# microsoft/vision-longformer

Hardware: NVIDIA H100
Metric: images/sec ViL-Small 224x224 training (higher is better)
Workload: dtype bf16

## Files before the change

### include/vil_attn.h

```cpp
#ifndef VIL_ATTN_H_
#define VIL_ATTN_H_

#include <stdint.h>

#ifdef __cplusplus
extern "C" {
#endif

#define VIL_ATTN_ABI_VERSION 3

enum { VIL_F32 = 0, VIL_BF16 = 1, VIL_F16 = 2 };

enum {
  VIL_IMPL_AUTO    = 0,
  VIL_IMPL_SIMT    = 1,
  VIL_IMPL_WGMMA   = 2
};

enum {
  VIL_FLAG_F32_OUT = 1,
  VIL_FLAG_UNFUSED = 2
};

enum {
  VIL_OK = 0,
  VIL_E_BADARG = -1,
  VIL_E_UNSUPPORTED = -2,
  VIL_E_CUDA = -3,
  VIL_E_WORKSPACE = -4
};

typedef struct VilTensor4 {
  void*   ptr;
  int64_t sb, sh, st;
} VilTensor4;

typedef struct VilAttnParams {
  int32_t struct_bytes;
  int32_t dtype;
  int32_t impl;
  int32_t B, H, D;
  int32_t nx, ny;
  int32_t w;
  int32_t nglo;
  int32_t exact;
  int32_t mode;
  float   scale;
  int32_t skip_mask;
  int32_t flags;

  VilTensor4 q;
  VilTensor4 k, v;
  VilTensor4 qg;
  VilTensor4 kg, vg;
  VilTensor4 o;
  VilTensor4 og;
  float* lse;
  float* lse_g;
  const float* bias_table;
  const float* g2l;
  const float* g2g;

  VilTensor4 d_o, d_og;
  VilTensor4 dq, dk, dv;
  VilTensor4 dqg;
  VilTensor4 dkg, dvg;
  float* d_bias_table;
  float* d_g2l;
  float* d_g2g;

  void*   workspace;
  int64_t workspace_bytes;

  float    dropout_p;
  uint32_t reserved2;
  uint64_t dropout_seed;
  uint64_t dropout_offset;
} VilAttnParams;

int         vil_attn_abi_version(void);
const char* vil_attn_last_error(void);
int64_t     vil_attn_launch_count(void);
const char* vil_attn_last_impl(void);
const char* vil_attn_last_kernel(void);

int64_t vil_attn_workspace_bytes(const VilAttnParams* p, int backward);

int vil_attn_wgmma_supported(const VilAttnParams* p);

int vil_attn_fwd_sm100(const VilAttnParams* p, void* stream);

int vil_attn_bwd_sm100(const VilAttnParams* p, void* stream);

typedef struct VilLayerNormParams {
  int32_t struct_bytes;
  int32_t x_dtype;
  int32_t y_dtype;
  int32_t C;
  int64_t rows;
  float   eps;
  int32_t reserved;
  const void*  x;
  const float* gamma;
  const float* beta;
  void*        y;
  float*       mean;
  float*       rstd;
  const void*  dy;
  void*        dx;
  float*       dgamma;
  float*       dbeta;
  void*        workspace;
  int64_t      workspace_bytes;
} VilLayerNormParams;

int64_t vil_layernorm_workspace_bytes(const VilLayerNormParams* p);
int vil_layernorm_fwd_sm100(const VilLayerNormParams* p, void* stream);
int vil_layernorm_bwd_sm100(const VilLayerNormParams* p, void* stream);

typedef struct VilAddNormParams {
  int32_t struct_bytes;
  int32_t b_dtype;
  int32_t y_dtype;
  int32_t C;
  int64_t rows;
  int64_t rows_per_sample;
  float   eps;
  int32_t reserved;
  const float* x;
  const void*  br;
  const float* bias;
  const float* rowscale;
  const float* gamma;
  const float* beta;
  float*       xo;
  void*        y;
  float*       mean;
  float*       rstd;
  const void*  dy;
  const float* gres;
  float*       dx;
  void*        dbr;
  float*       dgamma;
  float*       dbeta;
  float*       dbias;
  void*        workspace;
  int64_t      workspace_bytes;
} VilAddNormParams;

int64_t vil_addnorm_workspace_bytes(const VilAddNormParams* p);
int vil_addnorm_fwd_sm100(const VilAddNormParams* p, void* stream);
int vil_addnorm_bwd_sm100(const VilAddNormParams* p, void* stream);

enum { VIL_ACT_NONE = 0, VIL_ACT_GELU = 1 };
typedef struct VilBiasActParams {
  int32_t struct_bytes;
  int32_t dtype;
  int32_t C;
  int32_t act;
  int64_t rows;
  const void*  z;
  const float* bias;
  void*        a;
  const void*  da;
  void*        dz;
  float*       dbias;
  void*        workspace;
  int64_t      workspace_bytes;
} VilBiasActParams;

int64_t vil_bias_act_workspace_bytes(const VilBiasActParams* p);
int vil_bias_act_fwd_sm100(const VilBiasActParams* p, void* stream);
int vil_bias_act_bwd_sm100(const VilBiasActParams* p, void* stream);

#ifdef __cplusplus
}
#endif
#endif
```

### vision_longformer_b200/_lib.py

```python
from __future__ import annotations

import ctypes
import os
import threading

_HERE = os.path.dirname(os.path.abspath(__file__))
LIB_NAME = "libvil_attn.so"
LIB_PATH = os.environ.get("VIL_ATTN_LIB") or os.path.join(_HERE, LIB_NAME)

VIL_F32, VIL_BF16, VIL_F16 = 0, 1, 2
VIL_IMPL_AUTO, VIL_IMPL_SIMT, VIL_IMPL_WGMMA = 0, 1, 2
VIL_E_BADARG, VIL_E_UNSUPPORTED, VIL_E_CUDA, VIL_E_WORKSPACE = -1, -2, -3, -4
ABI_VERSION = 3
VIL_FLAG_F32_OUT, VIL_FLAG_UNFUSED = 1, 2

EXPORTS = (
    "vil_attn_abi_version", "vil_attn_last_error", "vil_attn_launch_count", "vil_attn_last_impl", "vil_attn_last_kernel",
    "vil_attn_workspace_bytes", "vil_attn_wgmma_supported", "vil_attn_fwd_sm100", "vil_attn_bwd_sm100",
    "vil_layernorm_workspace_bytes", "vil_layernorm_fwd_sm100", "vil_layernorm_bwd_sm100",
    "vil_addnorm_workspace_bytes", "vil_addnorm_fwd_sm100", "vil_addnorm_bwd_sm100",
    "vil_bias_act_workspace_bytes", "vil_bias_act_fwd_sm100", "vil_bias_act_bwd_sm100",
)
VIL_ACT_NONE, VIL_ACT_GELU = 0, 1


class VilTensor4(ctypes.Structure):
    _fields_ = [("ptr", ctypes.c_void_p), ("sb", ctypes.c_int64), ("sh", ctypes.c_int64), ("st", ctypes.c_int64)]


class VilAttnParams(ctypes.Structure):
    _fields_ = [
        ("struct_bytes", ctypes.c_int32), ("dtype", ctypes.c_int32), ("impl", ctypes.c_int32),
        ("B", ctypes.c_int32), ("H", ctypes.c_int32), ("D", ctypes.c_int32),
        ("nx", ctypes.c_int32), ("ny", ctypes.c_int32), ("w", ctypes.c_int32), ("nglo", ctypes.c_int32),
        ("exact", ctypes.c_int32), ("mode", ctypes.c_int32), ("scale", ctypes.c_float), ("skip_mask", ctypes.c_int32),
        ("flags", ctypes.c_int32),
        ("q", VilTensor4), ("k", VilTensor4), ("v", VilTensor4),
        ("qg", VilTensor4), ("kg", VilTensor4), ("vg", VilTensor4),
        ("o", VilTensor4), ("og", VilTensor4),
        ("lse", ctypes.c_void_p), ("lse_g", ctypes.c_void_p),
        ("bias_table", ctypes.c_void_p), ("g2l", ctypes.c_void_p), ("g2g", ctypes.c_void_p),
        ("d_o", VilTensor4), ("d_og", VilTensor4),
        ("dq", VilTensor4), ("dk", VilTensor4), ("dv", VilTensor4),
        ("dqg", VilTensor4), ("dkg", VilTensor4), ("dvg", VilTensor4),
        ("d_bias_table", ctypes.c_void_p), ("d_g2l", ctypes.c_void_p), ("d_g2g", ctypes.c_void_p),
        ("workspace", ctypes.c_void_p), ("workspace_bytes", ctypes.c_int64),
        ("dropout_p", ctypes.c_float), ("reserved2", ctypes.c_uint32),
        ("dropout_seed", ctypes.c_uint64), ("dropout_offset", ctypes.c_uint64),
    ]


class VilLayerNormParams(ctypes.Structure):
    _fields_ = [
        ("struct_bytes", ctypes.c_int32), ("x_dtype", ctypes.c_int32), ("y_dtype", ctypes.c_int32), ("C", ctypes.c_int32),
        ("rows", ctypes.c_int64), ("eps", ctypes.c_float), ("reserved", ctypes.c_int32),
        ("x", ctypes.c_void_p), ("gamma", ctypes.c_void_p), ("beta", ctypes.c_void_p),
        ("y", ctypes.c_void_p), ("mean", ctypes.c_void_p), ("rstd", ctypes.c_void_p),
        ("dy", ctypes.c_void_p), ("dx", ctypes.c_void_p), ("dgamma", ctypes.c_void_p), ("dbeta", ctypes.c_void_p),
        ("workspace", ctypes.c_void_p), ("workspace_bytes", ctypes.c_int64),
    ]


class VilAddNormParams(ctypes.Structure):
    _fields_ = [
        ("struct_bytes", ctypes.c_int32), ("b_dtype", ctypes.c_int32), ("y_dtype", ctypes.c_int32), ("C", ctypes.c_int32),
        ("rows", ctypes.c_int64), ("rows_per_sample", ctypes.c_int64), ("eps", ctypes.c_float), ("reserved", ctypes.c_int32),
        ("x", ctypes.c_void_p), ("br", ctypes.c_void_p), ("bias", ctypes.c_void_p), ("rowscale", ctypes.c_void_p),
        ("gamma", ctypes.c_void_p), ("beta", ctypes.c_void_p), ("xo", ctypes.c_void_p), ("y", ctypes.c_void_p),
        ("mean", ctypes.c_void_p), ("rstd", ctypes.c_void_p), ("dy", ctypes.c_void_p), ("gres", ctypes.c_void_p),
        ("dx", ctypes.c_void_p), ("dbr", ctypes.c_void_p), ("dgamma", ctypes.c_void_p), ("dbeta", ctypes.c_void_p),
        ("dbias", ctypes.c_void_p), ("workspace", ctypes.c_void_p), ("workspace_bytes", ctypes.c_int64),
    ]


class VilBiasActParams(ctypes.Structure):
    _fields_ = [
        ("struct_bytes", ctypes.c_int32), ("dtype", ctypes.c_int32), ("C", ctypes.c_int32), ("act", ctypes.c_int32),
        ("rows", ctypes.c_int64),
        ("z", ctypes.c_void_p), ("bias", ctypes.c_void_p), ("a", ctypes.c_void_p), ("da", ctypes.c_void_p),
        ("dz", ctypes.c_void_p), ("dbias", ctypes.c_void_p), ("workspace", ctypes.c_void_p), ("workspace_bytes", ctypes.c_int64),
    ]


_lib = None
_lock = threading.Lock()


def load() -> ctypes.CDLL:
    global _lib
    if _lib is not None:
        return _lib
    with _lock:
        if _lib is not None:
            return _lib
        if not os.path.exists(LIB_PATH):
            raise RuntimeError(
                f"{LIB_PATH} is missing: build it with `python -c 'import __graft_entry__ as g; g.build()'` "
                "(nvcc -gencode arch=compute_90a,code=sm_90a).  There is no CPU / PyTorch fallback.")
        lib = ctypes.CDLL(LIB_PATH)
        lib.vil_attn_abi_version.restype = ctypes.c_int
        lib.vil_attn_last_error.restype = ctypes.c_char_p
        lib.vil_attn_last_impl.restype = ctypes.c_char_p
        lib.vil_attn_last_kernel.restype = ctypes.c_char_p
        lib.vil_attn_launch_count.restype = ctypes.c_int64
        lib.vil_attn_workspace_bytes.restype = ctypes.c_int64
        lib.vil_attn_workspace_bytes.argtypes = [ctypes.POINTER(VilAttnParams), ctypes.c_int]
        lib.vil_attn_wgmma_supported.restype = ctypes.c_int
        lib.vil_attn_wgmma_supported.argtypes = [ctypes.POINTER(VilAttnParams)]
        for fn in (lib.vil_attn_fwd_sm100, lib.vil_attn_bwd_sm100):
            fn.restype = ctypes.c_int
            fn.argtypes = [ctypes.POINTER(VilAttnParams), ctypes.c_void_p]
        lib.vil_layernorm_workspace_bytes.restype = ctypes.c_int64
        lib.vil_layernorm_workspace_bytes.argtypes = [ctypes.POINTER(VilLayerNormParams)]
        for fn in (lib.vil_layernorm_fwd_sm100, lib.vil_layernorm_bwd_sm100):
            fn.restype = ctypes.c_int
            fn.argtypes = [ctypes.POINTER(VilLayerNormParams), ctypes.c_void_p]
        for ws, fns, st in ((lib.vil_addnorm_workspace_bytes, (lib.vil_addnorm_fwd_sm100, lib.vil_addnorm_bwd_sm100), VilAddNormParams),
                            (lib.vil_bias_act_workspace_bytes, (lib.vil_bias_act_fwd_sm100, lib.vil_bias_act_bwd_sm100), VilBiasActParams)):
            ws.restype = ctypes.c_int64
            ws.argtypes = [ctypes.POINTER(st)]
            for fn in fns:
                fn.restype = ctypes.c_int
                fn.argtypes = [ctypes.POINTER(st), ctypes.c_void_p]
        if lib.vil_attn_abi_version() != ABI_VERSION:
            raise RuntimeError(f"ABI mismatch: library {lib.vil_attn_abi_version()}, binding {ABI_VERSION}")
        _lib = lib
    return _lib


def last_error() -> str:
    return load().vil_attn_last_error().decode()


def last_impl() -> str:
    return load().vil_attn_last_impl().decode()


def last_kernel() -> str:
    return load().vil_attn_last_kernel().decode()


def launch_count() -> int:
    return int(load().vil_attn_launch_count())


def raise_for(code: int):
    if code == 0:
        return
    msg = last_error()
    if code == VIL_E_BADARG:
        raise ValueError(msg)
    if code == VIL_E_UNSUPPORTED:
        raise NotImplementedError(msg)
    raise RuntimeError(f"vil_attn error {code}: {msg}")
```

### vision_longformer_b200/csrc/vil_attn_api.cu

```cuda
#include <atomic>
#include <cmath>
#include <cstdarg>
#include <cstdio>
#include <cstring>

#include "vil_host.cuh"
#include "vil_layernorm.cuh"

namespace {

thread_local char g_err[512] = "";
thread_local const char* g_last_impl = "none";
thread_local const char* g_last_kernel = "";
std::atomic<long long> g_launches{0};

int fail(int code, const char* fmt, ...) {
  va_list ap;
  va_start(ap, fmt);
  vsnprintf(g_err, sizeof(g_err), fmt, ap);
  va_end(ap);
  return code;
}

#define VIL_CUDA_OK(expr)                                                                  \
  do {                                                                                     \
    cudaError_t e__ = (expr);                                                              \
    if (e__ != cudaSuccess) return fail(VIL_E_CUDA, "%s: %s", #expr, cudaGetErrorString(e__)); \
  } while (0)

#define VIL_LAUNCHED() g_launches.fetch_add(1, std::memory_order_relaxed)

int make_geo(const VilAttnParams* p, vil::Geo* g) {
  if (p == nullptr) return fail(VIL_E_BADARG, "params is NULL");
  if (p->struct_bytes != (int32_t)sizeof(VilAttnParams))
    return fail(VIL_E_BADARG, "VilAttnParams size mismatch: caller %d, library %d (ABI drift)", p->struct_bytes,
                (int)sizeof(VilAttnParams));
  if (p->dtype != VIL_F32 && p->dtype != VIL_BF16 && p->dtype != VIL_F16)
    return fail(VIL_E_BADARG, "dtype must be VIL_F32, VIL_BF16 or VIL_F16");
  if (p->B <= 0 || p->H <= 0 || p->D <= 0 || p->nx <= 0 || p->ny <= 0 || p->w <= 0 || p->nglo < 0)
    return fail(VIL_E_BADARG, "B, H, D, nx, ny, w must be positive and nglo non-negative");
  if (p->exact != 0 && p->exact != 1 && p->exact != -1)
    return fail(VIL_E_BADARG, "longsc exact should be in [0,1,-1]!");
  if (p->mode < -1 || p->mode > 8) return fail(VIL_E_BADARG, "mode must be in [-1, 8]");
  if (p->flags & ~(VIL_FLAG_F32_OUT | VIL_FLAG_UNFUSED)) return fail(VIL_E_BADARG, "unknown bits in flags");
  if ((p->flags & VIL_FLAG_F32_OUT) && p->dtype == VIL_F32)
    return fail(VIL_E_BADARG, "VIL_FLAG_F32_OUT is the parity build of the bf16 / fp16 kernels; dtype is already fp32");
  if (p->exact == 1 && p->mode != 0)
    return fail(VIL_E_BADARG, "exact sliding window (exact=1) only supports mode=0");
  if (p->D > 128) return fail(VIL_E_UNSUPPORTED, "head dim %d > 128 is not supported", p->D);
  if (p->w > 48) return fail(VIL_E_UNSUPPORTED, "window %d > 48 is not supported", p->w);
  if ((long long)p->nx * p->ny + p->nglo > 0x7fffffffLL / 4) return fail(VIL_E_UNSUPPORTED, "too many tokens");
  memset(g, 0, sizeof(*g));
  g->B = p->B; g->H = p->H; g->D = p->D;
  g->nx = p->nx; g->ny = p->ny; g->w = p->w; g->g = p->nglo; g->exact = p->exact; g->mode = p->mode;
  g->padx = (p->w - p->nx % p->w) % p->w;
  g->pady = (p->w - p->ny % p->w) % p->w;
  g->mx = (p->nx + g->padx) / p->w;
  g->my = (p->ny + g->pady) / p->w;
  g->Nloc = p->nx * p->ny;
  g->N = g->Nloc + p->nglo;
  g->w2 = p->w * p->w;
  g->npc = (g->w2 + 63) / 64;
  static const int o9[9][2] = {{-1, -1}, {-1, 0}, {-1, 1}, {0, -1}, {0, 0}, {0, 1}, {1, -1}, {1, 0}, {1, 1}};
  static const int om[9][2] = {{0, 0}, {-1, -1}, {-1, 0}, {-1, 1}, {0, -1}, {0, 1}, {1, -1}, {1, 0}, {1, 1}};
  if (p->mode == 0) {
    g->noffs = 9;
    for (int i = 0; i < 9; ++i) { g->offR[i] = o9[i][0]; g->offC[i] = o9[i][1]; }
  } else if (p->mode == -1) {
    g->noffs = 1;
  } else {
    g->noffs = 2;
    g->offR[1] = om[p->mode][0]; g->offC[1] = om[p->mode][1];
  }
  g->has_bias = p->bias_table != nullptr;
  g->scale = p->scale;
  if (g->has_bias && p->nglo > 0 && (p->g2l == nullptr || p->g2g == nullptr))
    return fail(VIL_E_BADARG, "bias_table given but g2l / g2g missing while nglo > 0");
  if (!g->has_bias && (p->g2l != nullptr || p->g2g != nullptr))
    return fail(VIL_E_BADARG, "g2l / g2g given without bias_table (rpe parameters come together)");
  if (!(p->dropout_p >= 0.f && p->dropout_p < 1.f))
    return fail(VIL_E_BADARG, "dropout_p must be in [0, 1) (got %g)", (double)p->dropout_p);
  g->drop_p = p->dropout_p;
  g->drop_scale = 1.0f / (1.0f - p->dropout_p);
  const double t = std::floor((double)p->dropout_p * 4294967296.0);
  g->drop_thresh = t >= 4294967295.0 ? 0xffffffffu : (uint32_t)t;
  g->seed_lo = (uint32_t)(p->dropout_seed & 0xffffffffu);
  g->seed_hi = (uint32_t)(p->dropout_seed >> 32);
  g->drop_off = (uint32_t)p->dropout_offset;
  return VIL_OK;
}

int check_tensor(const VilTensor4& t, const char* name) {
  if (t.ptr == nullptr) return fail(VIL_E_BADARG, "tensor %s is NULL", name);
  return VIL_OK;
}

int check_common(const VilAttnParams* p, const vil::Geo& g, bool bwd) {
  int rc;
  if ((rc = check_tensor(p->q, "q")) || (rc = check_tensor(p->k, "k")) || (rc = check_tensor(p->v, "v")) ||
      (rc = check_tensor(p->o, "o")))
    return rc;
  if (p->lse == nullptr) return fail(VIL_E_BADARG, "lse is NULL");
  if (g.g > 0) {
    if ((rc = check_tensor(p->qg, "qg")) || (rc = check_tensor(p->kg, "kg")) || (rc = check_tensor(p->vg, "vg")) ||
        (rc = check_tensor(p->og, "og")))
      return rc;
    if (p->lse_g == nullptr) return fail(VIL_E_BADARG, "lse_g is NULL");
  }
  if (bwd) {
    if ((rc = check_tensor(p->d_o, "d_o")) || (rc = check_tensor(p->dq, "dq")) || (rc = check_tensor(p->dk, "dk")) ||
        (rc = check_tensor(p->dv, "dv")))
      return rc;
    if (g.g > 0) {
      if ((rc = check_tensor(p->d_og, "d_og")) || (rc = check_tensor(p->dqg, "dqg"))) return rc;
      const bool shared = (p->kg.ptr == p->k.ptr) && (p->vg.ptr == p->v.ptr);
      if (!shared && ((rc = check_tensor(p->dkg, "dkg")) || (rc = check_tensor(p->dvg, "dvg")))) return rc;
    }
    const long long need = vil_attn_workspace_bytes(p, 1);
    if (p->workspace == nullptr || p->workspace_bytes < need)
      return fail(VIL_E_WORKSPACE, "workspace too small: need %lld bytes, got %lld", need,
                  (long long)p->workspace_bytes);
    if (g.has_bias && p->d_bias_table == nullptr) return fail(VIL_E_BADARG, "bias_table given but d_bias_table is NULL");
  }
  return VIL_OK;
}

int run(const VilAttnParams* p, void* stream, bool bwd) {
  vil::Geo g;
  int rc = make_geo(p, &g);
  if (rc) return rc;
  if ((rc = check_common(p, g, bwd))) return rc;
  cudaStream_t s = static_cast<cudaStream_t>(stream);
  const int tc_ok = vil::tc_supported(p, g, bwd);
  int impl = p->impl;
  if (impl == VIL_IMPL_AUTO) impl = tc_ok ? VIL_IMPL_WGMMA : VIL_IMPL_SIMT;
  if (impl == VIL_IMPL_WGMMA) {
    if (!tc_ok) return fail(VIL_E_UNSUPPORTED, "the wgmma family does not cover this configuration: %s", vil::tc_why_not(p, g, bwd));
    rc = bwd ? vil::tc_backward(p, g, s) : vil::tc_forward(p, g, s);
    if (rc == VIL_OK) g_last_impl = "wgmma";
    return rc;
  }
  if (impl != VIL_IMPL_SIMT) return fail(VIL_E_BADARG, "impl must be VIL_IMPL_AUTO, _SIMT or _TCGEN05");
  rc = vil::simt_run(p, g, s, bwd);
  if (rc == VIL_OK) g_last_impl = "simt";
  return rc;
}

}

namespace vil {
int shared_fail(int code, const char* msg) { return fail(code, "%s", msg); }
void count_launch() { VIL_LAUNCHED(); }
void note_kernel(const char* name) { g_last_kernel = name; }
}

namespace {

constexpr int kSMs = 132;

inline int ln_bwd_grid(long long rows) {
  long long g = rows / (vil::ln::kWarpsPerCta * 16);
  if (g < kSMs) g = kSMs;
  if (g > kSMs * 8) g = kSMs * 8;
  return (int)g;
}

int ln_check(const VilLayerNormParams* p, bool bwd) {
  if (p == nullptr) return fail(VIL_E_BADARG, "params is NULL");
  if (p->struct_bytes != (int32_t)sizeof(VilLayerNormParams)) return fail(VIL_E_BADARG, "VilLayerNormParams size mismatch");
  if (p->C <= 0 || p->C > 1024) return fail(VIL_E_UNSUPPORTED, "LayerNorm supports 1 <= C <= 1024 (got %d)", p->C);
  if (p->rows < 0) return fail(VIL_E_BADARG, "rows must be >= 0");
  const bool same = p->x_dtype == p->y_dtype;
  const bool mixed = p->x_dtype == VIL_F32 && (p->y_dtype == VIL_BF16 || p->y_dtype == VIL_F16);
  const bool widen = (p->x_dtype == VIL_BF16 || p->x_dtype == VIL_F16) && p->y_dtype == VIL_F32;
  if (!(same || mixed || widen) || p->x_dtype < 0 || p->x_dtype > 2) return fail(VIL_E_UNSUPPORTED, "unsupported LayerNorm dtype pair");
  if (!p->x || !p->gamma || !p->beta || !p->mean || !p->rstd) return fail(VIL_E_BADARG, "LayerNorm: NULL tensor");
  if (!bwd && !p->y) return fail(VIL_E_BADARG, "LayerNorm: y is NULL");
  if (bwd) {
    if (!p->dy || !p->dx || !p->dgamma || !p->dbeta) return fail(VIL_E_BADARG, "LayerNorm backward: NULL tensor");
    if (!p->workspace || p->workspace_bytes < vil_layernorm_workspace_bytes(p))
      return fail(VIL_E_WORKSPACE, "LayerNorm workspace too small");
  }
  return VIL_OK;
}

template <typename TX, typename TY, int NPL>
int ln_launch(const VilLayerNormParams* p, cudaStream_t s, bool bwd) {
  if (p->rows == 0) return VIL_OK;
  if (!bwd) {
    long long ctas = (p->rows + vil::ln::kWarpsPerCta - 1) / vil::ln::kWarpsPerCta;
    if (ctas > kSMs * 8) ctas = kSMs * 8;
    vil::ln::layernorm_fwd<TX, TY, NPL><<<(unsigned)ctas, vil::ln::kWarpsPerCta * 32, 0, s>>>(
        static_cast<const TX*>(p->x), p->gamma, p->beta, static_cast<TY*>(p->y), p->mean, p->rstd, p->rows, p->C, p->eps);
    VIL_LAUNCHED();
  } else {
    float* partial = static_cast<float*>(p->workspace);
    const int grid = ln_bwd_grid(p->rows);
    vil::ln::layernorm_bwd<TX, TY, NPL><<<grid, vil::ln::kWarpsPerCta * 32, 0, s>>>(
        static_cast<const TY*>(p->dy), static_cast<const TX*>(p->x), p->gamma, p->mean, p->rstd, static_cast<TX*>(p->dx),
        partial, p->rows, p->C);
    VIL_LAUNCHED();
    vil::ln::layernorm_bwd_reduce<<<(2 * p->C + 31) / 32, 256, 0, s>>>(partial, p->dgamma, p->dbeta, grid, p->C);
    VIL_LAUNCHED();
  }
  VIL_CUDA_OK(cudaGetLastError());
  return VIL_OK;
}

template <typename TX, typename TY>
int ln_dispatch_c(const VilLayerNormParams* p, cudaStream_t s, bool bwd) {
  const int npl = (p->C + 31) / 32;
  if (npl <= 3) return ln_launch<TX, TY, 3>(p, s, bwd);
  if (npl <= 6) return ln_launch<TX, TY, 6>(p, s, bwd);
  if (npl <= 12) return ln_launch<TX, TY, 12>(p, s, bwd);
  if (npl <= 24) return ln_launch<TX, TY, 24>(p, s, bwd);
  return ln_launch<TX, TY, 32>(p, s, bwd);
}

int ln_run(const VilLayerNormParams* p, void* stream, bool bwd) {
  int rc = ln_check(p, bwd);
  if (rc) return rc;
  cudaStream_t s = static_cast<cudaStream_t>(stream);
  if (p->x_dtype == VIL_F32) {
    if (p->y_dtype == VIL_F32) return ln_dispatch_c<float, float>(p, s, bwd);
    if (p->y_dtype == VIL_BF16) return ln_dispatch_c<float, __nv_bfloat16>(p, s, bwd);
    return ln_dispatch_c<float, __half>(p, s, bwd);
  }
  if (p->x_dtype == VIL_BF16)
    return p->y_dtype == VIL_F32 ? ln_dispatch_c<__nv_bfloat16, float>(p, s, bwd) : ln_dispatch_c<__nv_bfloat16, __nv_bfloat16>(p, s, bwd);
  return p->y_dtype == VIL_F32 ? ln_dispatch_c<__half, float>(p, s, bwd) : ln_dispatch_c<__half, __half>(p, s, bwd);
}

}

extern "C" {

int64_t vil_layernorm_workspace_bytes(const VilLayerNormParams* p) {
  if (p == nullptr || p->C <= 0) return VIL_E_BADARG;
  return (int64_t)ln_bwd_grid(p->rows) * 2 * p->C * 4 + 256;
}
int vil_layernorm_fwd_sm100(const VilLayerNormParams* p, void* stream) { return ln_run(p, stream, false); }
int vil_layernorm_bwd_sm100(const VilLayerNormParams* p, void* stream) { return ln_run(p, stream, true); }

#ifdef VIL_TRACE
int vil_attn_debug_set_trace(void* dev_ptr) {
  long long* p = static_cast<long long*>(dev_ptr);
  return (int)cudaMemcpyToSymbol(g_vil_trace, &p, sizeof(p));
}
#endif

int vil_attn_abi_version(void) { return VIL_ATTN_ABI_VERSION; }
const char* vil_attn_last_error(void) { return g_err; }
int64_t vil_attn_launch_count(void) { return g_launches.load(std::memory_order_relaxed); }
const char* vil_attn_last_impl(void) { return g_last_impl; }
const char* vil_attn_last_kernel(void) { return g_last_kernel; }

int64_t vil_attn_workspace_bytes(const VilAttnParams* p, int backward) {
  vil::Geo g;
  int rc = make_geo(p, &g);
  if (rc) return rc;
  long long bytes = 256;
  if (backward) bytes += vil::ws_floats(g) * 4;
  return bytes;
}

int vil_attn_wgmma_supported(const VilAttnParams* p) {
  vil::Geo g;
  int rc = make_geo(p, &g);
  if (rc) return rc;
  return vil::tc_supported(p, g, false) ? 1 : 0;
}

int vil_attn_fwd_sm100(const VilAttnParams* p, void* stream) { return run(p, stream, false); }
int vil_attn_bwd_sm100(const VilAttnParams* p, void* stream) { return run(p, stream, true); }

}
```

### vision_longformer_b200/csrc/vil_common.cuh

```cuda
#pragma once
#include <cuda_runtime.h>
#include <cuda_bf16.h>
#include <cuda_fp16.h>
#include <stdint.h>
#include "../../include/vil_attn.h"

namespace vil {

struct Geo {
  int B, H, D;
  int nx, ny, w, g, exact, mode;
  int padx, pady, mx, my;
  int Nloc, N, w2;
  int npc;
  int noffs;
  int offR[9], offC[9];
  int has_bias;
  float scale;
  float drop_p, drop_scale;
  uint32_t drop_thresh;
  uint32_t seed_lo, seed_hi, drop_off;
};

inline long long ws_off_delta_g(const Geo& g) { return ((long long)g.B * g.H * g.Nloc + 63) & ~63LL; }
inline long long ws_floats(const Geo& g) { return ws_off_delta_g(g) + (((long long)g.B * g.H * g.g + 63) & ~63LL); }

struct T4 {
  char* p;
  long long sb, sh, st;
};

template <typename T> struct ElemTraits;
template <> struct ElemTraits<float> {
  static __device__ __forceinline__ float to_f(float x) { return x; }
  static __device__ __forceinline__ float from_f(float x) { return x; }
};
template <> struct ElemTraits<__nv_bfloat16> {
  static __device__ __forceinline__ float to_f(__nv_bfloat16 x) { return __bfloat162float(x); }
  static __device__ __forceinline__ __nv_bfloat16 from_f(float x) { return __float2bfloat16_rn(x); }
};
template <> struct ElemTraits<__half> {
  static __device__ __forceinline__ float to_f(__half x) { return __half2float(x); }
  static __device__ __forceinline__ __half from_f(float x) { return __float2half_rn(x); }
};

template <typename T>
__device__ __forceinline__ const T* row_ptr(const T4& t, int b, int h, long long tok) {
  return reinterpret_cast<const T*>(t.p) + (long long)b * t.sb + (long long)h * t.sh + tok * t.st;
}
template <typename T>
__device__ __forceinline__ T* row_ptr_w(const T4& t, int b, int h, long long tok) {
  return reinterpret_cast<T*>(t.p) + (long long)b * t.sb + (long long)h * t.sh + tok * t.st;
}

template <typename T, int CNT>
__device__ __forceinline__ void load_seg(const T* __restrict__ row, int c0, int D, float (&r)[CNT]) {
  constexpr int PER16 = 16 / (int)sizeof(T);
  if constexpr (CNT % PER16 == 0) {
    if (c0 + CNT <= D && ((reinterpret_cast<uintptr_t>(row + c0)) & 15) == 0) {
#pragma unroll
      for (int v = 0; v < CNT / PER16; ++v) {
        int4 raw = __ldg(reinterpret_cast<const int4*>(row + c0) + v);
        const T* e = reinterpret_cast<const T*>(&raw);
#pragma unroll
        for (int u = 0; u < PER16; ++u) r[v * PER16 + u] = ElemTraits<T>::to_f(e[u]);
      }
      return;
    }
  }
#pragma unroll
  for (int c = 0; c < CNT; ++c) r[c] = (c0 + c < D) ? ElemTraits<T>::to_f(row[c0 + c]) : 0.f;
}

template <typename T, int CNT>
__device__ __forceinline__ void store_seg(T* __restrict__ row, int c0, int D, const float (&r)[CNT]) {
  constexpr int PER16 = 16 / (int)sizeof(T);
  if constexpr (CNT % PER16 == 0) {
    if (c0 + CNT <= D && ((reinterpret_cast<uintptr_t>(row + c0)) & 15) == 0) {
#pragma unroll
      for (int v = 0; v < CNT / PER16; ++v) {
        int4 raw;
        T* e = reinterpret_cast<T*>(&raw);
#pragma unroll
        for (int u = 0; u < PER16; ++u) e[u] = ElemTraits<T>::from_f(r[v * PER16 + u]);
        reinterpret_cast<int4*>(row + c0)[v] = raw;
      }
      return;
    }
  }
#pragma unroll
  for (int c = 0; c < CNT; ++c)
    if (c0 + c < D) row[c0 + c] = ElemTraits<T>::from_f(r[c]);
}

__device__ __forceinline__ uint4 philox(const Geo& g, uint32_t c0, uint32_t c1, uint32_t c2) {
  uint32_t x0 = c0, x1 = c1, x2 = c2, x3 = g.drop_off, k0 = g.seed_lo, k1 = g.seed_hi;
#pragma unroll
  for (int r = 0; r < 10; ++r) {
    const uint32_t lo0 = 0xD2511F53u * x0, hi0 = __umulhi(0xD2511F53u, x0);
    const uint32_t lo1 = 0xCD9E8D57u * x2, hi1 = __umulhi(0xCD9E8D57u, x2);
    x0 = hi1 ^ x1 ^ k0; x1 = lo1; x2 = hi0 ^ x3 ^ k1; x3 = lo0;
    k0 += 0x9E3779B9u; k1 += 0xBB67AE85u;
  }
  return make_uint4(x0, x1, x2, x3);
}
__device__ __forceinline__ uint32_t philox_word(const uint4& x, uint32_t w) {
  return w == 0 ? x.x : w == 1 ? x.y : w == 2 ? x.z : x.w;
}
__device__ __forceinline__ bool drop_keep(const Geo& g, uint32_t row, uint32_t col, uint32_t sid) {
  return philox_word(philox(g, col >> 2, row, sid), col & 3) >= g.drop_thresh;
}
__device__ __forceinline__ void drop_keep2(const Geo& g, uint32_t row, uint32_t col, uint32_t sid, bool& k0, bool& k1) {
  const uint4 x = philox(g, col >> 2, row, sid);
  const uint32_t w = col & 3;
  k0 = philox_word(x, w) >= g.drop_thresh;
  const uint32_t u1 = w == 3 ? philox(g, (col >> 2) + 1, row, sid).x : philox_word(x, w + 1);
  k1 = u1 >= g.drop_thresh;
}

__device__ __forceinline__ float warp_sum(float v) {
#pragma unroll
  for (int o = 16; o > 0; o >>= 1) v += __shfl_xor_sync(0xffffffffu, v, o);
  return v;
}

}
```

### vision_longformer_b200/csrc/vil_sm90.cuh

```cuda
#pragma once
#include <cuda_bf16.h>
#include <cuda_fp16.h>
#include <stdint.h>

namespace sm90 {

__device__ __forceinline__ uint32_t smem_u32(const void* p) { return (uint32_t)__cvta_generic_to_shared(p); }

__host__ __device__ constexpr int core_off(int r, int c, int K) { return (((r >> 3) * (K >> 3) + (c >> 3)) << 6) + ((r & 7) << 3) + (c & 7); }

__device__ __forceinline__ uint64_t make_desc(uint32_t addr, uint32_t lbo, uint32_t sbo) {
  return (uint64_t)((addr >> 4) & 0x3FFF) | (uint64_t)(lbo >> 4) << 16 | (uint64_t)(sbo >> 4) << 32;
}
__device__ __forceinline__ uint64_t desc(const void* tile, int K, int k16) {
  return make_desc(smem_u32(tile) + k16 * 256, 128, (K >> 3) * 128);
}
__device__ __forceinline__ uint64_t desc_mn(const void* tile, int N, int k16) {
  return make_desc(smem_u32(tile) + k16 * N * 32, N * 16, 128);
}

__device__ __forceinline__ void cp_async16(void* dst, const void* src, int n) {
  asm volatile("cp.async.cg.shared.global [%0], [%1], 16, %2;" ::"r"(smem_u32(dst)), "l"(src), "r"(n) : "memory");
}
__device__ __forceinline__ void cp_async4(void* dst, const void* src) {
  asm volatile("cp.async.ca.shared.global [%0], [%1], 4;" ::"r"(smem_u32(dst)), "l"(src) : "memory");
}
__device__ __forceinline__ void cp_async_commit() { asm volatile("cp.async.commit_group;" ::: "memory"); }
template <int N>
__device__ __forceinline__ void cp_async_wait() { asm volatile("cp.async.wait_group %0;" ::"n"(N) : "memory"); }

__device__ __forceinline__ void wg_fence() { asm volatile("wgmma.fence.sync.aligned;" ::: "memory"); }
__device__ __forceinline__ void wg_commit() { asm volatile("wgmma.commit_group.sync.aligned;" ::: "memory"); }
__device__ __forceinline__ void wg_wait0() { asm volatile("wgmma.wait_group.sync.aligned 0;" ::: "memory"); }
__device__ __forceinline__ void fence_proxy_async() { asm volatile("fence.proxy.async.shared::cta;" ::: "memory"); }
template <int R>
__device__ __forceinline__ void reg_fence(float (&d)[R]) {
#pragma unroll
  for (int i = 0; i < R; ++i) asm volatile("" : "+f"(d[i])::"memory");
}

__device__ __forceinline__ void wgmma_ss_bf16_n16(float (&d)[8], uint64_t a, uint64_t b, uint32_t acc) {
  asm volatile(
      "{\n\t.reg .pred p;\n\tsetp.ne.b32 p, %10, 0;\n\t"
      "wgmma.mma_async.sync.aligned.m64n16k16.f32.bf16.bf16 {%0,%1,%2,%3,%4,%5,%6,%7}, %8, %9, p, 1, 1, 0, 0;\n\t}"
      : "+f"(d[0]), "+f"(d[1]), "+f"(d[2]), "+f"(d[3]), "+f"(d[4]), "+f"(d[5]), "+f"(d[6]), "+f"(d[7])
      : "l"(a), "l"(b), "r"(acc));
}
__device__ __forceinline__ void wgmma_rs_bf16_n16(float (&d)[8], const uint32_t (&a)[4], uint64_t b, uint32_t acc) {
  asm volatile(
      "{\n\t.reg .pred p;\n\tsetp.ne.b32 p, %13, 0;\n\t"
      "wgmma.mma_async.sync.aligned.m64n16k16.f32.bf16.bf16 {%0,%1,%2,%3,%4,%5,%6,%7}, {%8,%9,%10,%11}, %12, p, 1, 1, 1;\n\t}"
      : "+f"(d[0]), "+f"(d[1]), "+f"(d[2]), "+f"(d[3]), "+f"(d[4]), "+f"(d[5]), "+f"(d[6]), "+f"(d[7])
      : "r"(a[0]), "r"(a[1]), "r"(a[2]), "r"(a[3]), "l"(b), "r"(acc));
}
__device__ __forceinline__ void wgmma_ss_f16_n16(float (&d)[8], uint64_t a, uint64_t b, uint32_t acc) {
  asm volatile(
      "{\n\t.reg .pred p;\n\tsetp.ne.b32 p, %10, 0;\n\t"
      "wgmma.mma_async.sync.aligned.m64n16k16.f32.f16.f16 {%0,%1,%2,%3,%4,%5,%6,%7}, %8, %9, p, 1, 1, 0, 0;\n\t}"
      : "+f"(d[0]), "+f"(d[1]), "+f"(d[2]), "+f"(d[3]), "+f"(d[4]), "+f"(d[5]), "+f"(d[6]), "+f"(d[7])
      : "l"(a), "l"(b), "r"(acc));
}
__device__ __forceinline__ void wgmma_rs_f16_n16(float (&d)[8], const uint32_t (&a)[4], uint64_t b, uint32_t acc) {
  asm volatile(
      "{\n\t.reg .pred p;\n\tsetp.ne.b32 p, %13, 0;\n\t"
      "wgmma.mma_async.sync.aligned.m64n16k16.f32.f16.f16 {%0,%1,%2,%3,%4,%5,%6,%7}, {%8,%9,%10,%11}, %12, p, 1, 1, 1;\n\t}"
      : "+f"(d[0]), "+f"(d[1]), "+f"(d[2]), "+f"(d[3]), "+f"(d[4]), "+f"(d[5]), "+f"(d[6]), "+f"(d[7])
      : "r"(a[0]), "r"(a[1]), "r"(a[2]), "r"(a[3]), "l"(b), "r"(acc));
}
__device__ __forceinline__ void wgmma_ss_bf16_n32(float (&d)[16], uint64_t a, uint64_t b, uint32_t acc) {
  asm volatile(
      "{\n\t.reg .pred p;\n\tsetp.ne.b32 p, %18, 0;\n\t"
      "wgmma.mma_async.sync.aligned.m64n32k16.f32.bf16.bf16 {%0,%1,%2,%3,%4,%5,%6,%7,%8,%9,%10,%11,%12,%13,%14,%15}, %16, %17, p, 1, 1, 0, 0;\n\t}"
      : "+f"(d[0]), "+f"(d[1]), "+f"(d[2]), "+f"(d[3]), "+f"(d[4]), "+f"(d[5]), "+f"(d[6]), "+f"(d[7]), "+f"(d[8]), "+f"(d[9]), "+f"(d[10]), "+f"(d[11]), "+f"(d[12]), "+f"(d[13]), "+f"(d[14]), "+f"(d[15])
      : "l"(a), "l"(b), "r"(acc));
}
__device__ __forceinline__ void wgmma_rs_bf16_n32(float (&d)[16], const uint32_t (&a)[4], uint64_t b, uint32_t acc) {
  asm volatile(
      "{\n\t.reg .pred p;\n\tsetp.ne.b32 p, %21, 0;\n\t"
      "wgmma.mma_async.sync.aligned.m64n32k16.f32.bf16.bf16 {%0,%1,%2,%3,%4,%5,%6,%7,%8,%9,%10,%11,%12,%13,%14,%15}, {%16,%17,%18,%19}, %20, p, 1, 1, 1;\n\t}"
      : "+f"(d[0]), "+f"(d[1]), "+f"(d[2]), "+f"(d[3]), "+f"(d[4]), "+f"(d[5]), "+f"(d[6]), "+f"(d[7]), "+f"(d[8]), "+f"(d[9]), "+f"(d[10]), "+f"(d[11]), "+f"(d[12]), "+f"(d[13]), "+f"(d[14]), "+f"(d[15])
      : "r"(a[0]), "r"(a[1]), "r"(a[2]), "r"(a[3]), "l"(b), "r"(acc));
}
__device__ __forceinline__ void wgmma_ss_f16_n32(float (&d)[16], uint64_t a, uint64_t b, uint32_t acc) {
  asm volatile(
      "{\n\t.reg .pred p;\n\tsetp.ne.b32 p, %18, 0;\n\t"
      "wgmma.mma_async.sync.aligned.m64n32k16.f32.f16.f16 {%0,%1,%2,%3,%4,%5,%6,%7,%8,%9,%10,%11,%12,%13,%14,%15}, %16, %17, p, 1, 1, 0, 0;\n\t}"
      : "+f"(d[0]), "+f"(d[1]), "+f"(d[2]), "+f"(d[3]), "+f"(d[4]), "+f"(d[5]), "+f"(d[6]), "+f"(d[7]), "+f"(d[8]), "+f"(d[9]), "+f"(d[10]), "+f"(d[11]), "+f"(d[12]), "+f"(d[13]), "+f"(d[14]), "+f"(d[15])
      : "l"(a), "l"(b), "r"(acc));
}
__device__ __forceinline__ void wgmma_rs_f16_n32(float (&d)[16], const uint32_t (&a)[4], uint64_t b, uint32_t acc) {
  asm volatile(
      "{\n\t.reg .pred p;\n\tsetp.ne.b32 p, %21, 0;\n\t"
      "wgmma.mma_async.sync.aligned.m64n32k16.f32.f16.f16 {%0,%1,%2,%3,%4,%5,%6,%7,%8,%9,%10,%11,%12,%13,%14,%15}, {%16,%17,%18,%19}, %20, p, 1, 1, 1;\n\t}"
      : "+f"(d[0]), "+f"(d[1]), "+f"(d[2]), "+f"(d[3]), "+f"(d[4]), "+f"(d[5]), "+f"(d[6]), "+f"(d[7]), "+f"(d[8]), "+f"(d[9]), "+f"(d[10]), "+f"(d[11]), "+f"(d[12]), "+f"(d[13]), "+f"(d[14]), "+f"(d[15])
      : "r"(a[0]), "r"(a[1]), "r"(a[2]), "r"(a[3]), "l"(b), "r"(acc));
}
__device__ __forceinline__ void wgmma_ss_bf16_n64(float (&d)[32], uint64_t a, uint64_t b, uint32_t acc) {
  asm volatile(
      "{\n\t.reg .pred p;\n\tsetp.ne.b32 p, %34, 0;\n\t"
      "wgmma.mma_async.sync.aligned.m64n64k16.f32.bf16.bf16 {%0,%1,%2,%3,%4,%5,%6,%7,%8,%9,%10,%11,%12,%13,%14,%15,%16,%17,%18,%19,%20,%21,%22,%23,%24,%25,%26,%27,%28,%29,%30,%31}, %32, %33, p, 1, 1, 0, 0;\n\t}"
      : "+f"(d[0]), "+f"(d[1]), "+f"(d[2]), "+f"(d[3]), "+f"(d[4]), "+f"(d[5]), "+f"(d[6]), "+f"(d[7]), "+f"(d[8]), "+f"(d[9]), "+f"(d[10]), "+f"(d[11]), "+f"(d[12]), "+f"(d[13]), "+f"(d[14]), "+f"(d[15]), "+f"(d[16]), "+f"(d[17]), "+f"(d[18]), "+f"(d[19]), "+f"(d[20]), "+f"(d[21]), "+f"(d[22]), "+f"(d[23]), "+f"(d[24]), "+f"(d[25]), "+f"(d[26]), "+f"(d[27]), "+f"(d[28]), "+f"(d[29]), "+f"(d[30]), "+f"(d[31])
      : "l"(a), "l"(b), "r"(acc));
}
__device__ __forceinline__ void wgmma_rs_bf16_n64(float (&d)[32], const uint32_t (&a)[4], uint64_t b, uint32_t acc) {
  asm volatile(
      "{\n\t.reg .pred p;\n\tsetp.ne.b32 p, %37, 0;\n\t"
      "wgmma.mma_async.sync.aligned.m64n64k16.f32.bf16.bf16 {%0,%1,%2,%3,%4,%5,%6,%7,%8,%9,%10,%11,%12,%13,%14,%15,%16,%17,%18,%19,%20,%21,%22,%23,%24,%25,%26,%27,%28,%29,%30,%31}, {%32,%33,%34,%35}, %36, p, 1, 1, 1;\n\t}"
      : "+f"(d[0]), "+f"(d[1]), "+f"(d[2]), "+f"(d[3]), "+f"(d[4]), "+f"(d[5]), "+f"(d[6]), "+f"(d[7]), "+f"(d[8]), "+f"(d[9]), "+f"(d[10]), "+f"(d[11]), "+f"(d[12]), "+f"(d[13]), "+f"(d[14]), "+f"(d[15]), "+f"(d[16]), "+f"(d[17]), "+f"(d[18]), "+f"(d[19]), "+f"(d[20]), "+f"(d[21]), "+f"(d[22]), "+f"(d[23]), "+f"(d[24]), "+f"(d[25]), "+f"(d[26]), "+f"(d[27]), "+f"(d[28]), "+f"(d[29]), "+f"(d[30]), "+f"(d[31])
      : "r"(a[0]), "r"(a[1]), "r"(a[2]), "r"(a[3]), "l"(b), "r"(acc));
}
__device__ __forceinline__ void wgmma_ss_f16_n64(float (&d)[32], uint64_t a, uint64_t b, uint32_t acc) {
  asm volatile(
      "{\n\t.reg .pred p;\n\tsetp.ne.b32 p, %34, 0;\n\t"
      "wgmma.mma_async.sync.aligned.m64n64k16.f32.f16.f16 {%0,%1,%2,%3,%4,%5,%6,%7,%8,%9,%10,%11,%12,%13,%14,%15,%16,%17,%18,%19,%20,%21,%22,%23,%24,%25,%26,%27,%28,%29,%30,%31}, %32, %33, p, 1, 1, 0, 0;\n\t}"
      : "+f"(d[0]), "+f"(d[1]), "+f"(d[2]), "+f"(d[3]), "+f"(d[4]), "+f"(d[5]), "+f"(d[6]), "+f"(d[7]), "+f"(d[8]), "+f"(d[9]), "+f"(d[10]), "+f"(d[11]), "+f"(d[12]), "+f"(d[13]), "+f"(d[14]), "+f"(d[15]), "+f"(d[16]), "+f"(d[17]), "+f"(d[18]), "+f"(d[19]), "+f"(d[20]), "+f"(d[21]), "+f"(d[22]), "+f"(d[23]), "+f"(d[24]), "+f"(d[25]), "+f"(d[26]), "+f"(d[27]), "+f"(d[28]), "+f"(d[29]), "+f"(d[30]), "+f"(d[31])
      : "l"(a), "l"(b), "r"(acc));
}
__device__ __forceinline__ void wgmma_rs_f16_n64(float (&d)[32], const uint32_t (&a)[4], uint64_t b, uint32_t acc) {
  asm volatile(
      "{\n\t.reg .pred p;\n\tsetp.ne.b32 p, %37, 0;\n\t"
      "wgmma.mma_async.sync.aligned.m64n64k16.f32.f16.f16 {%0,%1,%2,%3,%4,%5,%6,%7,%8,%9,%10,%11,%12,%13,%14,%15,%16,%17,%18,%19,%20,%21,%22,%23,%24,%25,%26,%27,%28,%29,%30,%31}, {%32,%33,%34,%35}, %36, p, 1, 1, 1;\n\t}"
      : "+f"(d[0]), "+f"(d[1]), "+f"(d[2]), "+f"(d[3]), "+f"(d[4]), "+f"(d[5]), "+f"(d[6]), "+f"(d[7]), "+f"(d[8]), "+f"(d[9]), "+f"(d[10]), "+f"(d[11]), "+f"(d[12]), "+f"(d[13]), "+f"(d[14]), "+f"(d[15]), "+f"(d[16]), "+f"(d[17]), "+f"(d[18]), "+f"(d[19]), "+f"(d[20]), "+f"(d[21]), "+f"(d[22]), "+f"(d[23]), "+f"(d[24]), "+f"(d[25]), "+f"(d[26]), "+f"(d[27]), "+f"(d[28]), "+f"(d[29]), "+f"(d[30]), "+f"(d[31])
      : "r"(a[0]), "r"(a[1]), "r"(a[2]), "r"(a[3]), "l"(b), "r"(acc));
}

template <typename T, int N> struct Wg;
#define VIL_WG(T, TN, N)                                                                                          \
  template <> struct Wg<T, N> {                                                                                   \
    static __device__ __forceinline__ void ss(float (&d)[N / 2], uint64_t a, uint64_t b, uint32_t acc) { wgmma_ss_##TN##_n##N(d, a, b, acc); } \
    static __device__ __forceinline__ void rs(float (&d)[N / 2], const uint32_t (&a)[4], uint64_t b, uint32_t acc) { wgmma_rs_##TN##_n##N(d, a, b, acc); } \
  };
VIL_WG(__nv_bfloat16, bf16, 16)
VIL_WG(__nv_bfloat16, bf16, 32)
VIL_WG(__nv_bfloat16, bf16, 64)
VIL_WG(__half, f16, 16)
VIL_WG(__half, f16, 32)
VIL_WG(__half, f16, 64)
#undef VIL_WG

template <typename T> __device__ __forceinline__ uint32_t pack2(float x, float y);
template <> __device__ __forceinline__ uint32_t pack2<__nv_bfloat16>(float x, float y) {
  __nv_bfloat162 v = __floats2bfloat162_rn(x, y);
  return *reinterpret_cast<uint32_t*>(&v);
}
template <> __device__ __forceinline__ uint32_t pack2<__half>(float x, float y) {
  __half2 v = __floats2half2_rn(x, y);
  return *reinterpret_cast<uint32_t*>(&v);
}

}
```

### vision_longformer_b200/csrc/vil_wgmma.cuh

```cuda
#pragma once
#include "vil_common.cuh"
#include "vil_sm90.cuh"

namespace vil {
namespace wg {

constexpr int kThreads = 128;

struct Cta { int b, h, R, C, piece; };

__device__ __forceinline__ Cta decode(const Geo& g, int bid) {
  Cta c;
  c.piece = bid % g.npc; bid /= g.npc;
  c.C = bid % g.my; bid /= g.my;
  c.R = bid % g.mx; bid /= g.mx;
  c.h = bid % g.H;
  c.b = bid / g.H;
  return c;
}

__device__ __forceinline__ int acc_row(int i) { return ((threadIdx.x >> 5) << 4) + ((threadIdx.x & 31) >> 2) + (((i >> 1) & 1) << 3); }
__device__ __forceinline__ int acc_col(int i) { return ((i >> 2) << 3) + ((threadIdx.x & 3) << 1) + (i & 1); }

constexpr int kStages = 3;

template <typename T, int HD>
__device__ __forceinline__ void stage_row(T* tile, const T* base, long long st, long long tok, int row, int half, int D) {
  constexpr int HH = HD / 2;
  const T* src = base + (tok < 0 ? 0 : tok * st);
#pragma unroll
  for (int g8 = 0; g8 < HH / 8; ++g8) {
    const int c = half * HH + g8 * 8;
    const bool in = tok >= 0 && c < D;
    sm90::cp_async16(tile + sm90::core_off(row, c, HD), in ? src + c : base, in ? 16 : 0);
  }
}

template <typename T>
__device__ __forceinline__ void to_a_frag(const float (&s)[32], int kk, uint32_t (&a)[4]) {
  a[0] = sm90::pack2<T>(s[8 * kk + 0], s[8 * kk + 1]);
  a[1] = sm90::pack2<T>(s[8 * kk + 2], s[8 * kk + 3]);
  a[2] = sm90::pack2<T>(s[8 * kk + 4], s[8 * kk + 5]);
  a[3] = sm90::pack2<T>(s[8 * kk + 6], s[8 * kk + 7]);
}

template <typename TO, int HD>
__device__ __forceinline__ void store_rows(const float (&acc)[HD / 2], int e, TO* row, int D, float mul) {
  const int c0 = (threadIdx.x & 3) << 1;
#pragma unroll
  for (int j = 0; j < HD / 8; ++j) {
    const int col = 8 * j + c0;
    if (col < D) row[col] = ElemTraits<TO>::from_f(acc[4 * j + 2 * e] * mul);
    if (col + 1 < D) row[col + 1] = ElemTraits<TO>::from_f(acc[4 * j + 2 * e + 1] * mul);
  }
}

__device__ __forceinline__ void drop_key_piece(float (&x)[32], const Geo& geo, const uint32_t (&row)[2], int cbase, uint32_t sid,
                                               float mul) {
  uint32_t keep = 0;
#pragma unroll 1
  for (int i = 0; i < 32; i += 2) {
    bool k0, k1;
    drop_keep2(geo, (i & 2) ? row[1] : row[0], (uint32_t)(cbase + acc_col(i)), sid, k0, k1);
    keep |= ((uint32_t)k0 | ((uint32_t)k1 << 1)) << i;
  }
#pragma unroll
  for (int i = 0; i < 32; ++i) x[i] = (keep >> i) & 1u ? x[i] * mul : 0.f;
}

__device__ __forceinline__ void drop_rows(const Geo& geo, int R, int C, int piece, uint32_t (&row)[2]) {
#pragma unroll
  for (int e = 0; e < 2; ++e) {
    const int l = piece * 64 + acc_row(2 * e);
    row[e] = (uint32_t)((R * geo.w + l / geo.w) * geo.ny + C * geo.w + l % geo.w);
  }
}

struct Visit {
  int r, c;
  int dR, dC;
  int cut;
  int oi;
};

__device__ __forceinline__ int visit_list(const Geo& geo, int R, int C, int sgn, Visit* vl) {
  int n = 0;
  for (int oi = 0; oi < geo.noffs; ++oi) {
    const int dR = geo.offR[oi], dC = geo.offC[oi];
    int r = R + sgn * dR, c = C + sgn * dC;
    if (geo.exact == -1) { r = (r + geo.mx) % geo.mx; c = (c + geo.my) % geo.my; }
    else if (r < 0 || r >= geo.mx || c < 0 || c >= geo.my) continue;
    const int qR = sgn > 0 ? R : r, qC = sgn > 0 ? C : c;
    if (threadIdx.x == 0) vl[n] = Visit{r, c, dR, dC, (qR + dR == geo.mx - 1) | ((qC + dC == geo.my - 1) << 1), oi};
    ++n;
  }
  return n;
}

__device__ __forceinline__ int drop_col_base(const Geo& geo, const Visit* vl, int ngp, int pi) {
  if (pi < ngp) return pi * 64;
  const int vi = (pi - ngp) / geo.npc;
  return geo.g + vl[vi].oi * geo.w2 + (pi - ngp - vi * geo.npc) * 64;
}

struct SlotWalk {
  int vi, pj, kr, kc;
  int r0, c0, dr, dc;
  __device__ __forceinline__ SlotWalk(const Geo& geo, int slot)
      : vi(0), pj(0), r0(slot / geo.w), c0(slot % geo.w), dr(64 / geo.w), dc(64 % geo.w) { kr = r0; kc = c0; }
  __device__ __forceinline__ void next(const Geo& geo) {
    if (++pj == geo.npc) { pj = 0; ++vi; kr = r0; kc = c0; return; }
    kr += dr; kc += dc;
    if (kc >= geo.w) { kc -= geo.w; ++kr; }
  }
};

__device__ __forceinline__ void chunk_key(const Geo& geo, const Visit& v, int kr, int kc, long long& tok, bool& ok, int& vr, int& vc) {
  const int w = geo.w;
  const int ar = v.r * w + kr, ac = v.c * w + kc;
  const bool real = (ar < geo.nx) && (ac < geo.ny);
  if (geo.exact == -1)
    ok = !(((v.cut & 1) && (kr >= w - geo.padx)) || ((v.cut & 2) && (kc >= w - geo.pady)));
  else
    ok = real;
  tok = (ok && real) ? geo.g + (long long)ar * geo.ny + ac : -1;
  vr = v.dR * w + kr; vc = v.dC * w + kc;
}

__device__ __forceinline__ void key_slot(const Geo& geo, const Visit* vl, int ngp, int pi, int slot, SlotWalk& wk, int& gk,
                                         long long& tok, bool& ok, int& vr, int& vc) {
  gk = -1; tok = -1; ok = false; vr = 0; vc = 0;
  if (pi < ngp) {
    const int t = pi * 64 + slot;
    if (t < geo.g) { gk = t; tok = t; ok = true; }
    return;
  }
  if (wk.kr < geo.w) chunk_key(geo, vl[wk.vi], wk.kr, wk.kc, tok, ok, vr, vc);
  wk.next(geo);
}

struct KeyCols {
  float* bias;
  int* tix;
  short* kr;
  short* kc;
};
struct QRows {
  int qr[2], qc[2];
  bool ok[2];
};

__device__ __forceinline__ QRows query_rows(const Geo& geo, int R, int C, int piece) {
  QRows q;
  const int w = geo.w;
#pragma unroll
  for (int e = 0; e < 2; ++e) {
    const int l = piece * 64 + acc_row(2 * e);
    const bool in = l < geo.w2;
    q.qr[e] = in ? l / w : 0; q.qc[e] = in ? l % w : 0;
    q.ok[e] = in && (R * w + q.qr[e] < geo.nx) && (C * w + q.qc[e] < geo.ny);
  }
  return q;
}

__device__ __forceinline__ void stage_key_cols(const Geo& geo, const KeyCols& kc, int h, const float* __restrict__ g2l, int gk,
                                               bool ok, int vr, int vc) {
  const int slot = threadIdx.x >> 1;
  float bias = ok ? 0.f : -INFINITY;
  if (gk >= 0 && geo.has_bias) bias = g2l[((long long)geo.H + h) * geo.g + gk];
  kc.bias[slot] = bias;
  kc.tix[slot] = vr * (4 * geo.w - 1) + vc;
  kc.kr[slot] = (short)vr;
  kc.kc[slot] = (short)vc;
}

__device__ __forceinline__ void row_tix(const Geo& geo, const QRows& q, int (&tb)[2]) {
  const int w = geo.w, tw = 4 * w - 1;
  tb[0] = (q.qr[0] + 2 * w - 1) * tw + q.qc[0] + 2 * w - 1;
  tb[1] = (q.qr[1] + 2 * w - 1) * tw + q.qc[1] + 2 * w - 1;
}

template <bool RPE, bool WIN>
__device__ __forceinline__ float key_score(const Geo& geo, const KeyCols& kc, const float* tab, const QRows& q, const int (&tb)[2],
                                           int e, int j, int gl, float s, int& bidx) {
  float bias = kc.bias[j];
  bidx = -1;
  if (RPE && j >= gl) { bidx = tb[e] - kc.tix[j]; bias += tab[bidx]; }
  if (WIN && (abs(q.qr[e] - kc.kr[j]) > geo.w || abs(q.qc[e] - kc.kc[j]) > geo.w)) return -INFINITY;
  return fmaf(geo.scale, s, bias);
}

__device__ __forceinline__ int key_epilogue(const Geo& geo) { return (geo.has_bias ? 2 : 0) | (geo.exact == 1 ? 1 : 0); }

template <bool RPE, bool WIN>
__device__ __forceinline__ void fwd_scores(float (&s)[32], float (&mx)[2], const Geo& geo, const KeyCols& kc, const float* tab,
                                           const QRows& q, int gl) {
  int tb[2] = {0, 0};
  if (RPE) row_tix(geo, q, tb);
#pragma unroll
  for (int i = 0; i < 32; ++i) {
    const int e = (i >> 1) & 1;
    int bidx;
    s[i] = key_score<RPE, WIN>(geo, kc, tab, q, tb, e, acc_col(i), gl, s[i], bidx);
    mx[e] = fmaxf(mx[e], s[i]);
  }
}

template <bool RPE, bool WIN>
__device__ __forceinline__ void dq_scores(float (&s)[32], const float (&dp)[32], const Geo& geo, const KeyCols& kc,
                                          const float* tab, const QRows& q, int gl, const float (&lse_r)[2],
                                          const float (&del_r)[2], float* __restrict__ d_table, int h) {
  int tb[2] = {0, 0};
  if (RPE) row_tix(geo, q, tb);
#pragma unroll
  for (int i = 0; i < 32; ++i) {
    const int e = (i >> 1) & 1;
    int bidx;
    const float val = key_score<RPE, WIN>(geo, kc, tab, q, tb, e, acc_col(i), gl, s[i], bidx);
    const float ds = __expf(val - lse_r[e]) * (dp[i] - del_r[e]);
    if (RPE && d_table != nullptr && bidx >= 0 && q.ok[e] && val != -INFINITY)
      atomicAdd(d_table + (long long)bidx * geo.H + h, ds);
    s[i] = ds;
  }
}

constexpr size_t kKeyCols = 64 * (4 + 4 + 2 + 2);
constexpr size_t kQueryCols = 64 * (4 + 4 + 4 + 2 + 2 + 1);
constexpr size_t kVisits = 9 * sizeof(Visit);
__host__ __device__ constexpr size_t query_cols_bytes(bool drop) { return kQueryCols + (drop ? 64 * sizeof(int) : 0); }

__device__ __forceinline__ KeyCols key_cols(unsigned char* meta, int stage) {
  KeyCols kc;
  kc.bias = reinterpret_cast<float*>(meta + stage * kKeyCols);
  kc.tix = reinterpret_cast<int*>(kc.bias + 64);
  kc.kr = reinterpret_cast<short*>(kc.tix + 64);
  kc.kc = kc.kr + 64;
  return kc;
}

template <int HD> struct FwdSmem {
  static constexpr size_t tiles = (1 + 2 * kStages) * 64 * HD * 2;
  static size_t total(int tabn) { return (tiles + kStages * kKeyCols + kVisits + (size_t)tabn * 4 + 15) & ~size_t(15); }
};
template <int HD> struct DqSmem {
  static constexpr size_t tiles = (2 + 2 * kStages) * 64 * HD * 2;
  static size_t total(int tabn) { return (tiles + kStages * kKeyCols + kVisits + (size_t)tabn * 4 + 15) & ~size_t(15); }
};
template <int HD> struct DkvSmem {
  static constexpr size_t tiles = (2 + 2 * kStages) * 64 * HD * 2;
  static size_t total(int tabn, bool drop = false) {
    return (tiles + kStages * query_cols_bytes(drop) + kVisits + 64 * sizeof(int) + (size_t)tabn * 4 + 15) & ~size_t(15);
  }
};

template <typename T, int HD>
__device__ __forceinline__ void issue_key_piece(const Geo& geo, int pi, int npieces, int ngp, const Visit* vl, SlotWalk& wk,
                                                T* ring, unsigned char* meta, const T* kb, long long kst, const T* vb,
                                                long long vst, int h, const float* __restrict__ g2l) {
  if (pi < npieces) {
    const int slot = threadIdx.x >> 1, half = threadIdx.x & 1, st = pi % kStages;
    int gk, vr, vc;
    long long tok;
    bool ok;
    key_slot(geo, vl, ngp, pi, slot, wk, gk, tok, ok, vr, vc);
    T* Ks = ring + st * 2 * 64 * HD;
    stage_row<T, HD>(Ks, kb, kst, tok, slot, half, geo.D);
    stage_row<T, HD>(Ks + 64 * HD, vb, vst, tok, slot, half, geo.D);
    if (half == 0) stage_key_cols(geo, key_cols(meta, st), h, g2l, gk, ok, vr, vc);
  }
  sm90::cp_async_commit();
}

__device__ __forceinline__ void ring_wait() {
  sm90::cp_async_wait<kStages - 2>();
  sm90::fence_proxy_async();
  __syncthreads();
}

template <typename T, int HD, typename TO, bool DROP = false>
__global__ void __launch_bounds__(kThreads, HD <= 32 ? 5 : 3)
wg_fwd_local(Geo geo, T4 q, T4 k, T4 v, T4 o, float* __restrict__ lse, const float* __restrict__ table,
             const float* __restrict__ g2l) {
  constexpr int HH = HD / 2, TILE = 64 * HD;
  using W64 = sm90::Wg<T, 64>;
  using WHD = sm90::Wg<T, HD>;
  extern __shared__ __align__(128) unsigned char smem_raw[];
  T* Qs = reinterpret_cast<T*>(smem_raw);
  T* ring = Qs + TILE;
  unsigned char* meta = reinterpret_cast<unsigned char*>(ring + 2 * kStages * TILE);
  Visit* vl = reinterpret_cast<Visit*>(meta + kStages * kKeyCols);
  float* tab = reinterpret_cast<float*>(vl + 9);
  const int tabn = geo.has_bias ? (4 * geo.w - 1) * (4 * geo.w - 1) : 0;

  const Cta cid = decode(geo, blockIdx.x);
  const int b = cid.b, h = cid.h, R = cid.R, C = cid.C;
  const int tid = threadIdx.x, slot = tid >> 1, half = tid & 1;
  const int w = geo.w, D = geo.D;
  for (int i = tid; i < tabn; i += kThreads) tab[i] = table[(long long)i * geo.H + h];
  {
    const int l = cid.piece * 64 + slot;
    const int r = R * w + l / w, c = C * w + l % w;
    const bool real = l < geo.w2 && r < geo.nx && c < geo.ny;
    stage_row<T, HD>(Qs, row_ptr<T>(q, b, h, 0), q.st, real ? (long long)r * geo.ny + c : -1, slot, half, D);
  }
  float m[2] = {-INFINITY, -INFINITY}, lsum[2] = {0.f, 0.f};
  float oacc[HH];
#pragma unroll
  for (int i = 0; i < HH; ++i) oacc[i] = 0.f;

  const int ngp = (geo.g + 63) / 64, npieces = ngp + visit_list(geo, R, C, 1, vl) * geo.npc;
  const int epi = key_epilogue(geo);
  const T* kb = row_ptr<T>(k, b, h, 0);
  const T* vb = row_ptr<T>(v, b, h, 0);
  SlotWalk wk(geo, slot);
  __syncthreads();
#pragma unroll
  for (int p = 0; p < kStages - 1; ++p)
    issue_key_piece<T, HD>(geo, p, npieces, ngp, vl, wk, ring, meta, kb, k.st, vb, v.st, h, g2l);
  for (int pi = 0; pi < npieces; ++pi) {
    ring_wait();
    issue_key_piece<T, HD>(geo, pi + kStages - 1, npieces, ngp, vl, wk, ring, meta, kb, k.st, vb, v.st, h, g2l);
    const int st = pi % kStages;
    const T* Ks = ring + st * 2 * TILE;
    const T* Vs = Ks + TILE;
    const KeyCols kcol = key_cols(meta, st);
    float s[32];
    sm90::wg_fence();
#pragma unroll
    for (int kk = 0; kk < HD / 16; ++kk) W64::ss(s, sm90::desc(Qs, HD, kk), sm90::desc(Ks, HD, kk), kk > 0);
    sm90::wg_commit();
    sm90::wg_wait0();
    sm90::reg_fence(s);
    float mx[2] = {-INFINITY, -INFINITY};
    const int gl = geo.g - pi * 64;
    switch (epi) {
      case 0: fwd_scores<false, false>(s, mx, geo, kcol, tab, query_rows(geo, R, C, cid.piece), gl); break;
      case 1: fwd_scores<false, true>(s, mx, geo, kcol, tab, query_rows(geo, R, C, cid.piece), gl); break;
      case 2: fwd_scores<true, false>(s, mx, geo, kcol, tab, query_rows(geo, R, C, cid.piece), gl); break;
      default: fwd_scores<true, true>(s, mx, geo, kcol, tab, query_rows(geo, R, C, cid.piece), gl); break;
    }
    float corr[2];
#pragma unroll
    for (int e = 0; e < 2; ++e) {
      mx[e] = fmaxf(mx[e], __shfl_xor_sync(0xffffffffu, mx[e], 1));
      mx[e] = fmaxf(mx[e], __shfl_xor_sync(0xffffffffu, mx[e], 2));
      const float mn = fmaxf(m[e], mx[e]);
      corr[e] = (mn == -INFINITY) ? 1.f : __expf(m[e] - mn);
      m[e] = mn;
      lsum[e] *= corr[e];
    }
#pragma unroll
    for (int i = 0; i < 32; ++i) {
      const int e = (i >> 1) & 1;
      const float p = (m[e] == -INFINITY) ? 0.f : __expf(s[i] - m[e]);
      s[i] = p;
      lsum[e] += p;
    }
#pragma unroll
    for (int i = 0; i < HH; ++i) oacc[i] *= corr[(i >> 1) & 1];
    if constexpr (DROP) {
      uint32_t drow[2];
      drop_rows(geo, R, C, cid.piece, drow);
      drop_key_piece(s, geo, drow, drop_col_base(geo, vl, ngp, pi), 2u * (uint32_t)(b * geo.H + h), 1.f);
    }
    uint32_t a[4][4];
#pragma unroll
    for (int kk = 0; kk < 4; ++kk) to_a_frag<T>(s, kk, a[kk]);
    sm90::wg_fence();
#pragma unroll
    for (int kk = 0; kk < 4; ++kk) WHD::rs(oacc, a[kk], sm90::desc_mn(Vs, HD, kk), 1);
    sm90::wg_commit();
    sm90::wg_wait0();
    sm90::reg_fence(oacc);
  }
  const QRows qrow = query_rows(geo, R, C, cid.piece);
#pragma unroll
  for (int e = 0; e < 2; ++e) {
    lsum[e] += __shfl_xor_sync(0xffffffffu, lsum[e], 1);
    lsum[e] += __shfl_xor_sync(0xffffffffu, lsum[e], 2);
    if (!qrow.ok[e]) continue;
    const long long tokq = (long long)(R * w + qrow.qr[e]) * geo.ny + (C * w + qrow.qc[e]);
    const float inv = lsum[e] > 0.f ? 1.f / lsum[e] : 0.f;
    store_rows<TO, HD>(oacc, e, row_ptr_w<TO>(o, b, h, tokq), D, DROP ? inv * geo.drop_scale : inv);
    if ((tid & 3) == 0) lse[((long long)b * geo.H + h) * geo.Nloc + tokq] = m[e] + logf(lsum[e]);
  }
}

template <typename T, int HD, typename TO, bool DROP = false>
__global__ void __launch_bounds__(kThreads)
wg_bwd_dq(Geo geo, T4 q, T4 k, T4 v, T4 d_o, T4 dq, const float* __restrict__ lse, const float* __restrict__ delta,
          const float* __restrict__ table, const float* __restrict__ g2l, float* __restrict__ d_table) {
  constexpr int HH = HD / 2, TILE = 64 * HD;
  using W64 = sm90::Wg<T, 64>;
  using WHD = sm90::Wg<T, HD>;
  extern __shared__ __align__(128) unsigned char smem_raw[];
  T* Qs = reinterpret_cast<T*>(smem_raw);
  T* Gs = Qs + TILE;
  T* ring = Gs + TILE;
  unsigned char* meta = reinterpret_cast<unsigned char*>(ring + 2 * kStages * TILE);
  Visit* vl = reinterpret_cast<Visit*>(meta + kStages * kKeyCols);
  float* tab = reinterpret_cast<float*>(vl + 9);
  const int tabn = geo.has_bias ? (4 * geo.w - 1) * (4 * geo.w - 1) : 0;

  const Cta cid = decode(geo, blockIdx.x);
  const int b = cid.b, h = cid.h, R = cid.R, C = cid.C;
  const int tid = threadIdx.x, slot = tid >> 1, half = tid & 1;
  const int w = geo.w, D = geo.D;
  const long long bh = (long long)b * geo.H + h;
  for (int i = tid; i < tabn; i += kThreads) tab[i] = table[(long long)i * geo.H + h];
  {
    const int l = cid.piece * 64 + slot;
    const int r = R * w + l / w, c = C * w + l % w;
    const long long tokq = (l < geo.w2 && r < geo.nx && c < geo.ny) ? (long long)r * geo.ny + c : -1;
    stage_row<T, HD>(Qs, row_ptr<T>(q, b, h, 0), q.st, tokq, slot, half, D);
    stage_row<T, HD>(Gs, row_ptr<T>(d_o, b, h, 0), d_o.st, tokq, slot, half, D);
  }
  const QRows qrow = query_rows(geo, R, C, cid.piece);
  float lse_r[2], del_r[2];
#pragma unroll
  for (int e = 0; e < 2; ++e) {
    lse_r[e] = INFINITY; del_r[e] = 0.f;
    if (qrow.ok[e]) {
      const long long tokq = (long long)(R * w + qrow.qr[e]) * geo.ny + (C * w + qrow.qc[e]);
      lse_r[e] = lse[bh * geo.Nloc + tokq];
      del_r[e] = delta[bh * geo.Nloc + tokq];
    }
  }
  float dqacc[HH];
#pragma unroll
  for (int i = 0; i < HH; ++i) dqacc[i] = 0.f;

  const int ngp = (geo.g + 63) / 64, npieces = ngp + visit_list(geo, R, C, 1, vl) * geo.npc;
  const int epi = key_epilogue(geo);
  const T* kb = row_ptr<T>(k, b, h, 0);
  const T* vb = row_ptr<T>(v, b, h, 0);
  SlotWalk wk(geo, slot);
  __syncthreads();
#pragma unroll
  for (int p = 0; p < kStages - 1; ++p)
    issue_key_piece<T, HD>(geo, p, npieces, ngp, vl, wk, ring, meta, kb, k.st, vb, v.st, h, g2l);
  for (int pi = 0; pi < npieces; ++pi) {
    ring_wait();
    issue_key_piece<T, HD>(geo, pi + kStages - 1, npieces, ngp, vl, wk, ring, meta, kb, k.st, vb, v.st, h, g2l);
    const int st = pi % kStages;
    const T* Ks = ring + st * 2 * TILE;
    const T* Vs = Ks + TILE;
    const KeyCols kcol = key_cols(meta, st);
    float s[32], dp[32];
    sm90::wg_fence();
#pragma unroll
    for (int kk = 0; kk < HD / 16; ++kk) W64::ss(s, sm90::desc(Qs, HD, kk), sm90::desc(Ks, HD, kk), kk > 0);
#pragma unroll
    for (int kk = 0; kk < HD / 16; ++kk) W64::ss(dp, sm90::desc(Gs, HD, kk), sm90::desc(Vs, HD, kk), kk > 0);
    sm90::wg_commit();
    sm90::wg_wait0();
    sm90::reg_fence(s);
    sm90::reg_fence(dp);
    const int gl = geo.g - pi * 64;
    if constexpr (DROP) {
      uint32_t drow[2];
      drop_rows(geo, R, C, cid.piece, drow);
      drop_key_piece(dp, geo, drow, drop_col_base(geo, vl, ngp, pi), 2u * (uint32_t)(b * geo.H + h), geo.drop_scale);
    }
    switch (epi) {
      case 0: dq_scores<false, false>(s, dp, geo, kcol, tab, qrow, gl, lse_r, del_r, d_table, h); break;
      case 1: dq_scores<false, true>(s, dp, geo, kcol, tab, qrow, gl, lse_r, del_r, d_table, h); break;
      case 2: dq_scores<true, false>(s, dp, geo, kcol, tab, qrow, gl, lse_r, del_r, d_table, h); break;
      default: dq_scores<true, true>(s, dp, geo, kcol, tab, qrow, gl, lse_r, del_r, d_table, h); break;
    }
    uint32_t a[4][4];
#pragma unroll
    for (int kk = 0; kk < 4; ++kk) to_a_frag<T>(s, kk, a[kk]);
    sm90::wg_fence();
#pragma unroll
    for (int kk = 0; kk < 4; ++kk) WHD::rs(dqacc, a[kk], sm90::desc_mn(Ks, HD, kk), 1);
    sm90::wg_commit();
    sm90::wg_wait0();
    sm90::reg_fence(dqacc);
  }
#pragma unroll
  for (int e = 0; e < 2; ++e) {
    if (!qrow.ok[e]) continue;
    const long long tokq = (long long)(R * w + qrow.qr[e]) * geo.ny + (C * w + qrow.qc[e]);
    store_rows<TO, HD>(dqacc, e, row_ptr_w<TO>(dq, b, h, tokq), D, geo.scale);
  }
}


struct QueryCols {
  float* lse;
  float* del;
  int* tix;
  short* qr;
  short* qc;
  unsigned char* cut;
  int* tok;
};
struct KRows {
  int kr[2], kc[2], tb[2];
  int cut[2];
  bool real[2];
};

__device__ __forceinline__ int key_pos(const Geo& geo, int piece, int row) {
  const int lk = piece * 64 + row;
  return lk < geo.w2 ? (lk / geo.w) | ((lk % geo.w) << 8) | (1 << 16) : 0;
}

__device__ __forceinline__ KRows key_rows(const Geo& geo, int KR, int KC, const int* kpos) {
  KRows k;
  const int w = geo.w, tw = 4 * w - 1;
#pragma unroll
  for (int e = 0; e < 2; ++e) {
    const int pos = kpos[acc_row(2 * e)];
    const bool in = pos >> 16;
    k.kr[e] = pos & 0xff; k.kc[e] = (pos >> 8) & 0xff;
    k.real[e] = in && (KR * w + k.kr[e] < geo.nx) && (KC * w + k.kc[e] < geo.ny);
    k.tb[e] = k.kr[e] * tw + k.kc[e] - (2 * w - 1) * (tw + 1);
    k.cut[e] = (k.kr[e] >= w - geo.padx) | ((k.kc[e] >= w - geo.pady) << 1);
  }
  return k;
}

__device__ __forceinline__ QueryCols query_cols(unsigned char* meta, int stage, int bytes) {
  QueryCols qc;
  qc.lse = reinterpret_cast<float*>(meta + stage * bytes);
  qc.del = qc.lse + 64;
  qc.tix = reinterpret_cast<int*>(qc.del + 64);
  qc.qr = reinterpret_cast<short*>(qc.tix + 64);
  qc.qc = qc.qr + 64;
  qc.cut = reinterpret_cast<unsigned char*>(qc.qc + 64);
  qc.tok = reinterpret_cast<int*>(qc.cut + 64);
  return qc;
}

template <typename T, int HD, bool DROP>
__device__ __forceinline__ void issue_query_piece(const Geo& geo, int qp, int npieces, const Visit* vl, SlotWalk& wk, T* ring,
                                                  unsigned char* meta, const T* qb, long long qst, const T* gb, long long gst,
                                                  const float* __restrict__ lse, const float* __restrict__ delta) {
  if (qp < npieces) {
    const int slot = threadIdx.x >> 1, half = threadIdx.x & 1, st = qp % kStages, w = geo.w;
    bool qv = false;
    long long tq = 0;
    int qa = 0, qb2 = 0, cut = 0;
    if (wk.kr < w) {
      const Visit vq = vl[wk.vi];
      const int r = vq.r * w + wk.kr, c = vq.c * w + wk.kc;
      qv = (r < geo.nx) && (c < geo.ny);
      tq = (long long)r * geo.ny + c;
      qa = wk.kr - vq.dR * w; qb2 = wk.kc - vq.dC * w; cut = vq.cut;
    }
    wk.next(geo);
    T* Qs = ring + st * 2 * 64 * HD;
    stage_row<T, HD>(Qs, qb, qst, qv ? tq : -1, slot, half, geo.D);
    stage_row<T, HD>(Qs + 64 * HD, gb, gst, qv ? tq : -1, slot, half, geo.D);
    if (half == 0) {
      const QueryCols qcol = query_cols(meta, st, (int)query_cols_bytes(DROP));
      if (qv) {
        sm90::cp_async4(qcol.lse + slot, lse + tq);
        sm90::cp_async4(qcol.del + slot, delta + tq);
      } else {
        qcol.lse[slot] = INFINITY;
        qcol.del[slot] = 0.f;
      }
      const int tw = 4 * w - 1;
      qcol.tix[slot] = qa * tw + qb2;
      qcol.qr[slot] = (short)qa; qcol.qc[slot] = (short)qb2;
      qcol.cut[slot] = (unsigned char)cut;
      if (DROP) qcol.tok[slot] = (int)tq;
    }
  }
  sm90::cp_async_commit();
}

__device__ __forceinline__ int query_epilogue(const Geo& geo) {
  return (geo.has_bias ? 3 : 0) + (geo.exact == 1 ? 1 : geo.exact == -1 ? 2 : 0);
}

template <bool RPE, int MASK>
__device__ __forceinline__ void dkv_probs(float (&s)[32], float (&dp)[32], const Geo& geo, const QueryCols& qc, const float* tab,
                                          const KRows& kr) {
#pragma unroll
  for (int i = 0; i < 32; ++i) {
    const int e = (i >> 1) & 1, j = acc_col(i);
    float x = fmaf(geo.scale, s[i], RPE ? tab[qc.tix[j] - kr.tb[e]] : 0.f) - qc.lse[j];
    if (MASK == 1 && (abs(qc.qr[j] - kr.kr[e]) > geo.w || abs(qc.qc[j] - kr.kc[e]) > geo.w)) x = -INFINITY;
    if (MASK == 2 && (qc.cut[j] & kr.cut[e])) x = -INFINITY;
    const float p = __expf(x);
    s[i] = p;
    dp[i] = p * (dp[i] - qc.del[j]);
  }
}

template <typename T, int HD, typename TO, bool DROP = false>
__global__ void __launch_bounds__(kThreads, (HD <= 32 ? 4 : 3) - (DROP ? 1 : 0))
wg_bwd_dkv(Geo geo, T4 q, T4 k, T4 v, T4 d_o, T4 dk, T4 dv, const float* __restrict__ lse, const float* __restrict__ delta,
           const float* __restrict__ table) {
  constexpr int HH = HD / 2, TILE = 64 * HD;
  using W64 = sm90::Wg<T, 64>;
  using WHD = sm90::Wg<T, HD>;
  extern __shared__ __align__(128) unsigned char smem_raw[];
  T* Ks = reinterpret_cast<T*>(smem_raw);
  T* Vs = Ks + TILE;
  T* ring = Vs + TILE;
  unsigned char* meta = reinterpret_cast<unsigned char*>(ring + 2 * kStages * TILE);
  const int cols = (int)query_cols_bytes(DROP);
  Visit* vl = reinterpret_cast<Visit*>(meta + kStages * cols);
  int* kpos = reinterpret_cast<int*>(vl + 9);
  float* tab = reinterpret_cast<float*>(kpos + 64);
  const int tw = 4 * geo.w - 1;
  const int tabn = geo.has_bias ? tw * tw : 0;

  const Cta cid = decode(geo, blockIdx.x);
  const int b = cid.b, h = cid.h, KR = cid.R, KC = cid.C;
  const int tid = threadIdx.x, slot = tid >> 1, half = tid & 1;
  const int w = geo.w, D = geo.D;
  const long long bh = (long long)b * geo.H + h;
  for (int i = tid; i < tabn; i += kThreads) tab[i] = table[(long long)i * geo.H + h];
  {
    const int lk = cid.piece * 64 + slot;
    const int ar = KR * w + lk / w, ac = KC * w + lk % w;
    const long long tokk = (lk < geo.w2 && ar < geo.nx && ac < geo.ny) ? geo.g + (long long)ar * geo.ny + ac : -1;
    stage_row<T, HD>(Ks, row_ptr<T>(k, b, h, 0), k.st, tokk, slot, half, D);
    stage_row<T, HD>(Vs, row_ptr<T>(v, b, h, 0), v.st, tokk, slot, half, D);
    if (half == 0) kpos[slot] = key_pos(geo, cid.piece, slot);
  }
  float dkacc[HH], dvacc[HH];
#pragma unroll
  for (int i = 0; i < HH; ++i) { dkacc[i] = 0.f; dvacc[i] = 0.f; }

  const int npieces = visit_list(geo, KR, KC, -1, vl) * geo.npc;
  const int epi = query_epilogue(geo);
  SlotWalk wk(geo, slot);
  __syncthreads();
#pragma unroll
  for (int p = 0; p < kStages - 1; ++p)
    issue_query_piece<T, HD, DROP>(geo, p, npieces, vl, wk, ring, meta, row_ptr<T>(q, b, h, 0), q.st,
                                   row_ptr<T>(d_o, b, h, 0), d_o.st, lse + bh * geo.Nloc, delta + bh * geo.Nloc);
  for (int qp = 0; qp < npieces; ++qp) {
    ring_wait();
    issue_query_piece<T, HD, DROP>(geo, qp + kStages - 1, npieces, vl, wk, ring, meta, row_ptr<T>(q, b, h, 0), q.st,
                                   row_ptr<T>(d_o, b, h, 0), d_o.st, lse + bh * geo.Nloc, delta + bh * geo.Nloc);
    const int st = qp % kStages;
    const T* Qs = ring + st * 2 * TILE;
    const T* Gs = Qs + TILE;
    const QueryCols qcol = query_cols(meta, st, cols);
    uint32_t keep = 0;
    if constexpr (DROP) {
      const int vi = qp / geo.npc;
      const uint32_t c0 = (uint32_t)(geo.g + vl[vi].oi * geo.w2 + cid.piece * 64), sid = 2u * (uint32_t)(b * geo.H + h);
#pragma unroll 1
      for (int i = 0; i < 32; ++i)
        keep |= (uint32_t)drop_keep(geo, (uint32_t)qcol.tok[acc_col(i)], c0 + (uint32_t)acc_row(i), sid) << i;
    }
    float s[32], dp[32];
    sm90::wg_fence();
#pragma unroll
    for (int kk = 0; kk < HD / 16; ++kk) W64::ss(s, sm90::desc(Ks, HD, kk), sm90::desc(Qs, HD, kk), kk > 0);
#pragma unroll
    for (int kk = 0; kk < HD / 16; ++kk) W64::ss(dp, sm90::desc(Vs, HD, kk), sm90::desc(Gs, HD, kk), kk > 0);
    sm90::wg_commit();
    sm90::wg_wait0();
    sm90::reg_fence(s);
    sm90::reg_fence(dp);
    if constexpr (DROP) {
#pragma unroll
      for (int i = 0; i < 32; ++i) dp[i] = (keep >> i) & 1u ? dp[i] * geo.drop_scale : 0.f;
    }
    switch (epi) {
      case 0: dkv_probs<false, 0>(s, dp, geo, qcol, tab, key_rows(geo, KR, KC, kpos)); break;
      case 1: dkv_probs<false, 1>(s, dp, geo, qcol, tab, key_rows(geo, KR, KC, kpos)); break;
      case 2: dkv_probs<false, 2>(s, dp, geo, qcol, tab, key_rows(geo, KR, KC, kpos)); break;
      case 3: dkv_probs<true, 0>(s, dp, geo, qcol, tab, key_rows(geo, KR, KC, kpos)); break;
      case 4: dkv_probs<true, 1>(s, dp, geo, qcol, tab, key_rows(geo, KR, KC, kpos)); break;
      default: dkv_probs<true, 2>(s, dp, geo, qcol, tab, key_rows(geo, KR, KC, kpos)); break;
    }
    if constexpr (DROP) {
#pragma unroll
      for (int i = 0; i < 32; ++i) s[i] = (keep >> i) & 1u ? s[i] * geo.drop_scale : 0.f;
    }
    uint32_t ap[4][4], ad[4][4];
#pragma unroll
    for (int kk = 0; kk < 4; ++kk) { to_a_frag<T>(s, kk, ap[kk]); to_a_frag<T>(dp, kk, ad[kk]); }
    sm90::wg_fence();
#pragma unroll
    for (int kk = 0; kk < 4; ++kk) WHD::rs(dvacc, ap[kk], sm90::desc_mn(Gs, HD, kk), 1);
#pragma unroll
    for (int kk = 0; kk < 4; ++kk) WHD::rs(dkacc, ad[kk], sm90::desc_mn(Qs, HD, kk), 1);
    sm90::wg_commit();
    sm90::wg_wait0();
    sm90::reg_fence(dvacc);
    sm90::reg_fence(dkacc);
  }
  const KRows krow = key_rows(geo, KR, KC, kpos);
#pragma unroll
  for (int e = 0; e < 2; ++e) {
    if (!krow.real[e]) continue;
    const long long tokk = geo.g + (long long)(KR * w + krow.kr[e]) * geo.ny + (KC * w + krow.kc[e]);
    store_rows<TO, HD>(dkacc, e, row_ptr_w<TO>(dk, b, h, tokk), D, geo.scale);
    store_rows<TO, HD>(dvacc, e, row_ptr_w<TO>(dv, b, h, tokk), D, 1.f);
  }
}

}
}
```

Before: 3805.

## Size wgmma N-width to actual piece width to skip padded columns

Adds wgmma ss variants for N=8 and N=56 and selects the MMA width per piece (global pieces, last partial pieces, windows of at most 56 tokens) instead of always using N=64. The padded rows and columns of the 64-wide tiles are no longer computed in the score and backward dK/dV GEMMs. It also trims the matching epilogue and dropout loops. A new FULL_PIECES flag restores the old fixed-64 behaviour. The change adds template instantiations and runtime switches, which raises code size and branch cost.

```diff
diff --git a/include/vil_attn.h b/include/vil_attn.h
--- a/include/vil_attn.h
+++ b/include/vil_attn.h
@@ -19,7 +19,8 @@
 
 enum {
   VIL_FLAG_F32_OUT = 1,
-  VIL_FLAG_UNFUSED = 2
+  VIL_FLAG_UNFUSED = 2,
+  VIL_FLAG_FULL_PIECES = 4
 };
 
 enum {
diff --git a/vision_longformer_b200/_lib.py b/vision_longformer_b200/_lib.py
--- a/vision_longformer_b200/_lib.py
+++ b/vision_longformer_b200/_lib.py
@@ -12,7 +12,7 @@
 VIL_IMPL_AUTO, VIL_IMPL_SIMT, VIL_IMPL_WGMMA = 0, 1, 2
 VIL_E_BADARG, VIL_E_UNSUPPORTED, VIL_E_CUDA, VIL_E_WORKSPACE = -1, -2, -3, -4
 ABI_VERSION = 3
-VIL_FLAG_F32_OUT, VIL_FLAG_UNFUSED = 1, 2
+VIL_FLAG_F32_OUT, VIL_FLAG_UNFUSED, VIL_FLAG_FULL_PIECES = 1, 2, 4
 
 EXPORTS = (
     "vil_attn_abi_version", "vil_attn_last_error", "vil_attn_launch_count", "vil_attn_last_impl", "vil_attn_last_kernel",
diff --git a/vision_longformer_b200/csrc/vil_attn_api.cu b/vision_longformer_b200/csrc/vil_attn_api.cu
--- a/vision_longformer_b200/csrc/vil_attn_api.cu
+++ b/vision_longformer_b200/csrc/vil_attn_api.cu
@@ -42,7 +42,7 @@
   if (p->exact != 0 && p->exact != 1 && p->exact != -1)
     return fail(VIL_E_BADARG, "longsc exact should be in [0,1,-1]!");
   if (p->mode < -1 || p->mode > 8) return fail(VIL_E_BADARG, "mode must be in [-1, 8]");
-  if (p->flags & ~(VIL_FLAG_F32_OUT | VIL_FLAG_UNFUSED)) return fail(VIL_E_BADARG, "unknown bits in flags");
+  if (p->flags & ~(VIL_FLAG_F32_OUT | VIL_FLAG_UNFUSED | VIL_FLAG_FULL_PIECES)) return fail(VIL_E_BADARG, "unknown bits in flags");
   if ((p->flags & VIL_FLAG_F32_OUT) && p->dtype == VIL_F32)
     return fail(VIL_E_BADARG, "VIL_FLAG_F32_OUT is the parity build of the bf16 / fp16 kernels; dtype is already fp32");
   if (p->exact == 1 && p->mode != 0)
@@ -73,6 +73,7 @@
     g->offR[1] = om[p->mode][0]; g->offC[1] = om[p->mode][1];
   }
   g->has_bias = p->bias_table != nullptr;
+  g->full_pieces = (p->flags & VIL_FLAG_FULL_PIECES) != 0;
   g->scale = p->scale;
   if (g->has_bias && p->nglo > 0 && (p->g2l == nullptr || p->g2g == nullptr))
     return fail(VIL_E_BADARG, "bias_table given but g2l / g2g missing while nglo > 0");
diff --git a/vision_longformer_b200/csrc/vil_common.cuh b/vision_longformer_b200/csrc/vil_common.cuh
--- a/vision_longformer_b200/csrc/vil_common.cuh
+++ b/vision_longformer_b200/csrc/vil_common.cuh
@@ -16,6 +16,7 @@
   int noffs;
   int offR[9], offC[9];
   int has_bias;
+  int full_pieces;
   float scale;
   float drop_p, drop_scale;
   uint32_t drop_thresh;
diff --git a/vision_longformer_b200/csrc/vil_sm90.cuh b/vision_longformer_b200/csrc/vil_sm90.cuh
--- a/vision_longformer_b200/csrc/vil_sm90.cuh
+++ b/vision_longformer_b200/csrc/vil_sm90.cuh
@@ -39,26 +39,52 @@
   for (int i = 0; i < R; ++i) asm volatile("" : "+f"(d[i])::"memory");
 }
 
-__device__ __forceinline__ void wgmma_ss_bf16_n16(float (&d)[8], uint64_t a, uint64_t b, uint32_t acc) {
-  asm volatile(
-      "{\n\t.reg .pred p;\n\tsetp.ne.b32 p, %10, 0;\n\t"
-      "wgmma.mma_async.sync.aligned.m64n16k16.f32.bf16.bf16 {%0,%1,%2,%3,%4,%5,%6,%7}, %8, %9, p, 1, 1, 0, 0;\n\t}"
-      : "+f"(d[0]), "+f"(d[1]), "+f"(d[2]), "+f"(d[3]), "+f"(d[4]), "+f"(d[5]), "+f"(d[6]), "+f"(d[7])
-      : "l"(a), "l"(b), "r"(acc));
-}
+#define VIL_ACC4(d, i) "+f"(d[i]), "+f"(d[i + 1]), "+f"(d[i + 2]), "+f"(d[i + 3])
+#define VIL_ACC_8(d) VIL_ACC4(d, 0)
+#define VIL_ACC_16(d) VIL_ACC_8(d), VIL_ACC4(d, 4)
+#define VIL_ACC_32(d) VIL_ACC_16(d), VIL_ACC4(d, 8), VIL_ACC4(d, 12)
+#define VIL_ACC_56(d) VIL_ACC_32(d), VIL_ACC4(d, 16), VIL_ACC4(d, 20), VIL_ACC4(d, 24)
+#define VIL_ACC_64(d) VIL_ACC_56(d), VIL_ACC4(d, 28)
+#define VIL_REG_8 "%3,%4,%5,%6"
+#define VIL_REG_16 VIL_REG_8 ",%7,%8,%9,%10"
+#define VIL_REG_32 VIL_REG_16 ",%11,%12,%13,%14,%15,%16,%17,%18"
+#define VIL_REG_56 VIL_REG_32 ",%19,%20,%21,%22,%23,%24,%25,%26,%27,%28,%29,%30"
+#define VIL_REG_64 VIL_REG_56 ",%31,%32,%33,%34"
+#define VIL_WGMMA_SS(TN, N)                                                                                         \
+  __device__ __forceinline__ void wgmma_ss_##TN##_n##N(float (&d)[N / 2], uint64_t a, uint64_t b, uint32_t acc) {  \
+    asm volatile("{\n\t.reg .pred p;\n\tsetp.ne.b32 p, %2, 0;\n\t"                                                 \
+                 "wgmma.mma_async.sync.aligned.m64n" #N "k16.f32." #TN "." #TN " {" VIL_REG_##N "}, %0, %1, p, 1, 1, 0, 0;\n\t}" \
+                 : "+l"(a), "+l"(b), "+r"(acc), VIL_ACC_##N(d));                                                    \
+  }
+VIL_WGMMA_SS(bf16, 8)
+VIL_WGMMA_SS(bf16, 16)
+VIL_WGMMA_SS(bf16, 32)
+VIL_WGMMA_SS(bf16, 56)
+VIL_WGMMA_SS(bf16, 64)
+VIL_WGMMA_SS(f16, 8)
+VIL_WGMMA_SS(f16, 16)
+VIL_WGMMA_SS(f16, 32)
+VIL_WGMMA_SS(f16, 56)
+VIL_WGMMA_SS(f16, 64)
+#undef VIL_WGMMA_SS
+#undef VIL_ACC4
+#undef VIL_ACC_8
+#undef VIL_ACC_16
+#undef VIL_ACC_32
+#undef VIL_ACC_56
+#undef VIL_ACC_64
+#undef VIL_REG_8
+#undef VIL_REG_16
+#undef VIL_REG_32
+#undef VIL_REG_56
+#undef VIL_REG_64
+
 __device__ __forceinline__ void wgmma_rs_bf16_n16(float (&d)[8], const uint32_t (&a)[4], uint64_t b, uint32_t acc) {
   asm volatile(
       "{\n\t.reg .pred p;\n\tsetp.ne.b32 p, %13, 0;\n\t"
       "wgmma.mma_async.sync.aligned.m64n16k16.f32.bf16.bf16 {%0,%1,%2,%3,%4,%5,%6,%7}, {%8,%9,%10,%11}, %12, p, 1, 1, 1;\n\t}"
       : "+f"(d[0]), "+f"(d[1]), "+f"(d[2]), "+f"(d[3]), "+f"(d[4]), "+f"(d[5]), "+f"(d[6]), "+f"(d[7])
       : "r"(a[0]), "r"(a[1]), "r"(a[2]), "r"(a[3]), "l"(b), "r"(acc));
-}
-__device__ __forceinline__ void wgmma_ss_f16_n16(float (&d)[8], uint64_t a, uint64_t b, uint32_t acc) {
-  asm volatile(
-      "{\n\t.reg .pred p;\n\tsetp.ne.b32 p, %10, 0;\n\t"
-      "wgmma.mma_async.sync.aligned.m64n16k16.f32.f16.f16 {%0,%1,%2,%3,%4,%5,%6,%7}, %8, %9, p, 1, 1, 0, 0;\n\t}"
-      : "+f"(d[0]), "+f"(d[1]), "+f"(d[2]), "+f"(d[3]), "+f"(d[4]), "+f"(d[5]), "+f"(d[6]), "+f"(d[7])
-      : "l"(a), "l"(b), "r"(acc));
 }
 __device__ __forceinline__ void wgmma_rs_f16_n16(float (&d)[8], const uint32_t (&a)[4], uint64_t b, uint32_t acc) {
   asm volatile(
@@ -67,26 +93,12 @@
       : "+f"(d[0]), "+f"(d[1]), "+f"(d[2]), "+f"(d[3]), "+f"(d[4]), "+f"(d[5]), "+f"(d[6]), "+f"(d[7])
       : "r"(a[0]), "r"(a[1]), "r"(a[2]), "r"(a[3]), "l"(b), "r"(acc));
 }
-__device__ __forceinline__ void wgmma_ss_bf16_n32(float (&d)[16], uint64_t a, uint64_t b, uint32_t acc) {
-  asm volatile(
-      "{\n\t.reg .pred p;\n\tsetp.ne.b32 p, %18, 0;\n\t"
-      "wgmma.mma_async.sync.aligned.m64n32k16.f32.bf16.bf16 {%0,%1,%2,%3,%4,%5,%6,%7,%8,%9,%10,%11,%12,%13,%14,%15}, %16, %17, p, 1, 1, 0, 0;\n\t}"
-      : "+f"(d[0]), "+f"(d[1]), "+f"(d[2]), "+f"(d[3]), "+f"(d[4]), "+f"(d[5]), "+f"(d[6]), "+f"(d[7]), "+f"(d[8]), "+f"(d[9]), "+f"(d[10]), "+f"(d[11]), "+f"(d[12]), "+f"(d[13]), "+f"(d[14]), "+f"(d[15])
-      : "l"(a), "l"(b), "r"(acc));
-}
 __device__ __forceinline__ void wgmma_rs_bf16_n32(float (&d)[16], const uint32_t (&a)[4], uint64_t b, uint32_t acc) {
   asm volatile(
       "{\n\t.reg .pred p;\n\tsetp.ne.b32 p, %21, 0;\n\t"
       "wgmma.mma_async.sync.aligned.m64n32k16.f32.bf16.bf16 {%0,%1,%2,%3,%4,%5,%6,%7,%8,%9,%10,%11,%12,%13,%14,%15}, {%16,%17,%18,%19}, %20, p, 1, 1, 1;\n\t}"
       : "+f"(d[0]), "+f"(d[1]), "+f"(d[2]), "+f"(d[3]), "+f"(d[4]), "+f"(d[5]), "+f"(d[6]), "+f"(d[7]), "+f"(d[8]), "+f"(d[9]), "+f"(d[10]), "+f"(d[11]), "+f"(d[12]), "+f"(d[13]), "+f"(d[14]), "+f"(d[15])
       : "r"(a[0]), "r"(a[1]), "r"(a[2]), "r"(a[3]), "l"(b), "r"(acc));
-}
-__device__ __forceinline__ void wgmma_ss_f16_n32(float (&d)[16], uint64_t a, uint64_t b, uint32_t acc) {
-  asm volatile(
-      "{\n\t.reg .pred p;\n\tsetp.ne.b32 p, %18, 0;\n\t"
-      "wgmma.mma_async.sync.aligned.m64n32k16.f32.f16.f16 {%0,%1,%2,%3,%4,%5,%6,%7,%8,%9,%10,%11,%12,%13,%14,%15}, %16, %17, p, 1, 1, 0, 0;\n\t}"
-      : "+f"(d[0]), "+f"(d[1]), "+f"(d[2]), "+f"(d[3]), "+f"(d[4]), "+f"(d[5]), "+f"(d[6]), "+f"(d[7]), "+f"(d[8]), "+f"(d[9]), "+f"(d[10]), "+f"(d[11]), "+f"(d[12]), "+f"(d[13]), "+f"(d[14]), "+f"(d[15])
-      : "l"(a), "l"(b), "r"(acc));
 }
 __device__ __forceinline__ void wgmma_rs_f16_n32(float (&d)[16], const uint32_t (&a)[4], uint64_t b, uint32_t acc) {
   asm volatile(
@@ -95,26 +107,12 @@
       : "+f"(d[0]), "+f"(d[1]), "+f"(d[2]), "+f"(d[3]), "+f"(d[4]), "+f"(d[5]), "+f"(d[6]), "+f"(d[7]), "+f"(d[8]), "+f"(d[9]), "+f"(d[10]), "+f"(d[11]), "+f"(d[12]), "+f"(d[13]), "+f"(d[14]), "+f"(d[15])
       : "r"(a[0]), "r"(a[1]), "r"(a[2]), "r"(a[3]), "l"(b), "r"(acc));
 }
-__device__ __forceinline__ void wgmma_ss_bf16_n64(float (&d)[32], uint64_t a, uint64_t b, uint32_t acc) {
-  asm volatile(
-      "{\n\t.reg .pred p;\n\tsetp.ne.b32 p, %34, 0;\n\t"
-      "wgmma.mma_async.sync.aligned.m64n64k16.f32.bf16.bf16 {%0,%1,%2,%3,%4,%5,%6,%7,%8,%9,%10,%11,%12,%13,%14,%15,%16,%17,%18,%19,%20,%21,%22,%23,%24,%25,%26,%27,%28,%29,%30,%31}, %32, %33, p, 1, 1, 0, 0;\n\t}"
-      : "+f"(d[0]), "+f"(d[1]), "+f"(d[2]), "+f"(d[3]), "+f"(d[4]), "+f"(d[5]), "+f"(d[6]), "+f"(d[7]), "+f"(d[8]), "+f"(d[9]), "+f"(d[10]), "+f"(d[11]), "+f"(d[12]), "+f"(d[13]), "+f"(d[14]), "+f"(d[15]), "+f"(d[16]), "+f"(d[17]), "+f"(d[18]), "+f"(d[19]), "+f"(d[20]), "+f"(d[21]), "+f"(d[22]), "+f"(d[23]), "+f"(d[24]), "+f"(d[25]), "+f"(d[26]), "+f"(d[27]), "+f"(d[28]), "+f"(d[29]), "+f"(d[30]), "+f"(d[31])
-      : "l"(a), "l"(b), "r"(acc));
-}
 __device__ __forceinline__ void wgmma_rs_bf16_n64(float (&d)[32], const uint32_t (&a)[4], uint64_t b, uint32_t acc) {
   asm volatile(
       "{\n\t.reg .pred p;\n\tsetp.ne.b32 p, %37, 0;\n\t"
       "wgmma.mma_async.sync.aligned.m64n64k16.f32.bf16.bf16 {%0,%1,%2,%3,%4,%5,%6,%7,%8,%9,%10,%11,%12,%13,%14,%15,%16,%17,%18,%19,%20,%21,%22,%23,%24,%25,%26,%27,%28,%29,%30,%31}, {%32,%33,%34,%35}, %36, p, 1, 1, 1;\n\t}"
       : "+f"(d[0]), "+f"(d[1]), "+f"(d[2]), "+f"(d[3]), "+f"(d[4]), "+f"(d[5]), "+f"(d[6]), "+f"(d[7]), "+f"(d[8]), "+f"(d[9]), "+f"(d[10]), "+f"(d[11]), "+f"(d[12]), "+f"(d[13]), "+f"(d[14]), "+f"(d[15]), "+f"(d[16]), "+f"(d[17]), "+f"(d[18]), "+f"(d[19]), "+f"(d[20]), "+f"(d[21]), "+f"(d[22]), "+f"(d[23]), "+f"(d[24]), "+f"(d[25]), "+f"(d[26]), "+f"(d[27]), "+f"(d[28]), "+f"(d[29]), "+f"(d[30]), "+f"(d[31])
       : "r"(a[0]), "r"(a[1]), "r"(a[2]), "r"(a[3]), "l"(b), "r"(acc));
-}
-__device__ __forceinline__ void wgmma_ss_f16_n64(float (&d)[32], uint64_t a, uint64_t b, uint32_t acc) {
-  asm volatile(
-      "{\n\t.reg .pred p;\n\tsetp.ne.b32 p, %34, 0;\n\t"
-      "wgmma.mma_async.sync.aligned.m64n64k16.f32.f16.f16 {%0,%1,%2,%3,%4,%5,%6,%7,%8,%9,%10,%11,%12,%13,%14,%15,%16,%17,%18,%19,%20,%21,%22,%23,%24,%25,%26,%27,%28,%29,%30,%31}, %32, %33, p, 1, 1, 0, 0;\n\t}"
-      : "+f"(d[0]), "+f"(d[1]), "+f"(d[2]), "+f"(d[3]), "+f"(d[4]), "+f"(d[5]), "+f"(d[6]), "+f"(d[7]), "+f"(d[8]), "+f"(d[9]), "+f"(d[10]), "+f"(d[11]), "+f"(d[12]), "+f"(d[13]), "+f"(d[14]), "+f"(d[15]), "+f"(d[16]), "+f"(d[17]), "+f"(d[18]), "+f"(d[19]), "+f"(d[20]), "+f"(d[21]), "+f"(d[22]), "+f"(d[23]), "+f"(d[24]), "+f"(d[25]), "+f"(d[26]), "+f"(d[27]), "+f"(d[28]), "+f"(d[29]), "+f"(d[30]), "+f"(d[31])
-      : "l"(a), "l"(b), "r"(acc));
 }
 __device__ __forceinline__ void wgmma_rs_f16_n64(float (&d)[32], const uint32_t (&a)[4], uint64_t b, uint32_t acc) {
   asm volatile(
@@ -125,18 +123,22 @@
 }
 
 template <typename T, int N> struct Wg;
-#define VIL_WG(T, TN, N)                                                                                          \
-  template <> struct Wg<T, N> {                                                                                   \
-    static __device__ __forceinline__ void ss(float (&d)[N / 2], uint64_t a, uint64_t b, uint32_t acc) { wgmma_ss_##TN##_n##N(d, a, b, acc); } \
-    static __device__ __forceinline__ void rs(float (&d)[N / 2], const uint32_t (&a)[4], uint64_t b, uint32_t acc) { wgmma_rs_##TN##_n##N(d, a, b, acc); } \
-  };
-VIL_WG(__nv_bfloat16, bf16, 16)
-VIL_WG(__nv_bfloat16, bf16, 32)
-VIL_WG(__nv_bfloat16, bf16, 64)
-VIL_WG(__half, f16, 16)
-VIL_WG(__half, f16, 32)
-VIL_WG(__half, f16, 64)
-#undef VIL_WG
+#define VIL_SS(TN, N) \
+  static __device__ __forceinline__ void ss(float (&d)[N / 2], uint64_t a, uint64_t b, uint32_t acc) { wgmma_ss_##TN##_n##N(d, a, b, acc); }
+#define VIL_RS(TN, N) \
+  static __device__ __forceinline__ void rs(float (&d)[N / 2], const uint32_t (&a)[4], uint64_t b, uint32_t acc) { wgmma_rs_##TN##_n##N(d, a, b, acc); }
+template <> struct Wg<__nv_bfloat16, 8> { VIL_SS(bf16, 8) };
+template <> struct Wg<__nv_bfloat16, 16> { VIL_SS(bf16, 16) VIL_RS(bf16, 16) };
+template <> struct Wg<__nv_bfloat16, 32> { VIL_SS(bf16, 32) VIL_RS(bf16, 32) };
+template <> struct Wg<__nv_bfloat16, 56> { VIL_SS(bf16, 56) };
+template <> struct Wg<__nv_bfloat16, 64> { VIL_SS(bf16, 64) VIL_RS(bf16, 64) };
+template <> struct Wg<__half, 8> { VIL_SS(f16, 8) };
+template <> struct Wg<__half, 16> { VIL_SS(f16, 16) VIL_RS(f16, 16) };
+template <> struct Wg<__half, 32> { VIL_SS(f16, 32) VIL_RS(f16, 32) };
+template <> struct Wg<__half, 56> { VIL_SS(f16, 56) };
+template <> struct Wg<__half, 64> { VIL_SS(f16, 64) VIL_RS(f16, 64) };
+#undef VIL_SS
+#undef VIL_RS
 
 template <typename T> __device__ __forceinline__ uint32_t pack2(float x, float y);
 template <> __device__ __forceinline__ uint32_t pack2<__nv_bfloat16>(float x, float y) {
diff --git a/vision_longformer_b200/csrc/vil_wgmma.cuh b/vision_longformer_b200/csrc/vil_wgmma.cuh
--- a/vision_longformer_b200/csrc/vil_wgmma.cuh
+++ b/vision_longformer_b200/csrc/vil_wgmma.cuh
@@ -36,13 +36,27 @@
   }
 }
 
-template <typename T>
-__device__ __forceinline__ void to_a_frag(const float (&s)[32], int kk, uint32_t (&a)[4]) {
+template <typename T, int NW>
+__device__ __forceinline__ void to_a_frag(const float (&s)[NW / 2], int kk, uint32_t (&a)[4]) {
   a[0] = sm90::pack2<T>(s[8 * kk + 0], s[8 * kk + 1]);
   a[1] = sm90::pack2<T>(s[8 * kk + 2], s[8 * kk + 3]);
-  a[2] = sm90::pack2<T>(s[8 * kk + 4], s[8 * kk + 5]);
-  a[3] = sm90::pack2<T>(s[8 * kk + 6], s[8 * kk + 7]);
-}
+  if (8 * kk + 4 < NW / 2) {
+    a[2] = sm90::pack2<T>(s[8 * kk + 4], s[8 * kk + 5]);
+    a[3] = sm90::pack2<T>(s[8 * kk + 6], s[8 * kk + 7]);
+  } else {
+    a[2] = 0u;
+    a[3] = 0u;
+  }
+}
+
+__device__ __forceinline__ int piece_width(int n) { return n <= 8 ? 8 : n <= 56 ? 56 : 64; }
+
+#define VIL_BY_WIDTH(nw, ROUND)                                                                                      \
+  switch (nw) {                                                                                                      \
+    case 8: ROUND(8); break;                                                                                         \
+    case 56: ROUND(56); break;                                                                                       \
+    default: ROUND(64); break;                                                                                       \
+  }
 
 template <typename TO, int HD>
 __device__ __forceinline__ void store_rows(const float (&acc)[HD / 2], int e, TO* row, int D, float mul) {
@@ -55,17 +69,18 @@
   }
 }
 
-__device__ __forceinline__ void drop_key_piece(float (&x)[32], const Geo& geo, const uint32_t (&row)[2], int cbase, uint32_t sid,
-                                               float mul) {
+template <int NW>
+__device__ __forceinline__ void drop_key_piece(float (&x)[NW / 2], const Geo& geo, const uint32_t (&row)[2], int cbase,
+                                               uint32_t sid, float mul) {
   uint32_t keep = 0;
 #pragma unroll 1
-  for (int i = 0; i < 32; i += 2) {
+  for (int i = 0; i < NW / 2; i += 2) {
     bool k0, k1;
     drop_keep2(geo, (i & 2) ? row[1] : row[0], (uint32_t)(cbase + acc_col(i)), sid, k0, k1);
     keep |= ((uint32_t)k0 | ((uint32_t)k1 << 1)) << i;
   }
 #pragma unroll
-  for (int i = 0; i < 32; ++i) x[i] = (keep >> i) & 1u ? x[i] * mul : 0.f;
+  for (int i = 0; i < NW / 2; ++i) x[i] = (keep >> i) & 1u ? x[i] * mul : 0.f;
 }
 
 __device__ __forceinline__ void drop_rows(const Geo& geo, int R, int C, int piece, uint32_t (&row)[2]) {
@@ -115,6 +130,11 @@
   }
 };
 
+__device__ __forceinline__ int issue_width(const Geo& geo, int pi, int ngp, const SlotWalk& wk) {
+  const int n = pi < ngp ? min(64, geo.g - 64 * pi) : wk.pj == geo.npc - 1 ? geo.w2 - 64 * (geo.npc - 1) : 64;
+  return geo.full_pieces ? 64 : piece_width(n);
+}
+
 __device__ __forceinline__ void chunk_key(const Geo& geo, const Visit& v, int kr, int kc, long long& tok, bool& ok, int& vr, int& vc) {
   const int w = geo.w;
   const int ar = v.r * w + kr, ac = v.c * w + kc;
@@ -192,13 +212,13 @@
 
 __device__ __forceinline__ int key_epilogue(const Geo& geo) { return (geo.has_bias ? 2 : 0) | (geo.exact == 1 ? 1 : 0); }
 
-template <bool RPE, bool WIN>
-__device__ __forceinline__ void fwd_scores(float (&s)[32], float (&mx)[2], const Geo& geo, const KeyCols& kc, const float* tab,
-                                           const QRows& q, int gl) {
+template <bool RPE, bool WIN, int NW>
+__device__ __forceinline__ void fwd_scores(float (&s)[NW / 2], float (&mx)[2], const Geo& geo, const KeyCols& kc,
+                                           const float* tab, const QRows& q, int gl) {
   int tb[2] = {0, 0};
   if (RPE) row_tix(geo, q, tb);
 #pragma unroll
-  for (int i = 0; i < 32; ++i) {
+  for (int i = 0; i < NW / 2; ++i) {
     const int e = (i >> 1) & 1;
     int bidx;
     s[i] = key_score<RPE, WIN>(geo, kc, tab, q, tb, e, acc_col(i), gl, s[i], bidx);
@@ -206,14 +226,14 @@
   }
 }
 
-template <bool RPE, bool WIN>
-__device__ __forceinline__ void dq_scores(float (&s)[32], const float (&dp)[32], const Geo& geo, const KeyCols& kc,
+template <bool RPE, bool WIN, int NW>
+__device__ __forceinline__ void dq_scores(float (&s)[NW / 2], const float (&dp)[NW / 2], const Geo& geo, const KeyCols& kc,
                                           const float* tab, const QRows& q, int gl, const float (&lse_r)[2],
                                           const float (&del_r)[2], float* __restrict__ d_table, int h) {
   int tb[2] = {0, 0};
   if (RPE) row_tix(geo, q, tb);
 #pragma unroll
-  for (int i = 0; i < 32; ++i) {
+  for (int i = 0; i < NW / 2; ++i) {
     const int e = (i >> 1) & 1;
     int bidx;
     const float val = key_score<RPE, WIN>(geo, kc, tab, q, tb, e, acc_col(i), gl, s[i], bidx);
@@ -227,6 +247,7 @@
 constexpr size_t kKeyCols = 64 * (4 + 4 + 2 + 2);
 constexpr size_t kQueryCols = 64 * (4 + 4 + 4 + 2 + 2 + 1);
 constexpr size_t kVisits = 9 * sizeof(Visit);
+constexpr size_t kWidths = kStages * sizeof(int);
 __host__ __device__ constexpr size_t query_cols_bytes(bool drop) { return kQueryCols + (drop ? 64 * sizeof(int) : 0); }
 
 __device__ __forceinline__ KeyCols key_cols(unsigned char* meta, int stage) {
@@ -240,11 +261,11 @@
 
 template <int HD> struct FwdSmem {
   static constexpr size_t tiles = (1 + 2 * kStages) * 64 * HD * 2;
-  static size_t total(int tabn) { return (tiles + kStages * kKeyCols + kVisits + (size_t)tabn * 4 + 15) & ~size_t(15); }
+  static size_t total(int tabn) { return (tiles + kStages * kKeyCols + kVisits + kWidths + (size_t)tabn * 4 + 15) & ~size_t(15); }
 };
 template <int HD> struct DqSmem {
   static constexpr size_t tiles = (2 + 2 * kStages) * 64 * HD * 2;
-  static size_t total(int tabn) { return (tiles + kStages * kKeyCols + kVisits + (size_t)tabn * 4 + 15) & ~size_t(15); }
+  static size_t total(int tabn) { return (tiles + kStages * kKeyCols + kVisits + kWidths + (size_t)tabn * 4 + 15) & ~size_t(15); }
 };
 template <int HD> struct DkvSmem {
   static constexpr size_t tiles = (2 + 2 * kStages) * 64 * HD * 2;
@@ -253,20 +274,22 @@
   }
 };
 
-template <typename T, int HD>
+template <typename T, int HD, bool KRS, bool TRIM = true>
 __device__ __forceinline__ void issue_key_piece(const Geo& geo, int pi, int npieces, int ngp, const Visit* vl, SlotWalk& wk,
-                                                T* ring, unsigned char* meta, const T* kb, long long kst, const T* vb,
-                                                long long vst, int h, const float* __restrict__ g2l) {
+                                                int* widths, T* ring, unsigned char* meta, const T* kb, long long kst,
+                                                const T* vb, long long vst, int h, const float* __restrict__ g2l) {
   if (pi < npieces) {
     const int slot = threadIdx.x >> 1, half = threadIdx.x & 1, st = pi % kStages;
+    const int nw = TRIM ? issue_width(geo, pi, ngp, wk) : 64, nrs = (nw + 15) & ~15;
+    if (threadIdx.x == 0) widths[st] = nw;
     int gk, vr, vc;
     long long tok;
     bool ok;
     key_slot(geo, vl, ngp, pi, slot, wk, gk, tok, ok, vr, vc);
     T* Ks = ring + st * 2 * 64 * HD;
-    stage_row<T, HD>(Ks, kb, kst, tok, slot, half, geo.D);
-    stage_row<T, HD>(Ks + 64 * HD, vb, vst, tok, slot, half, geo.D);
-    if (half == 0) stage_key_cols(geo, key_cols(meta, st), h, g2l, gk, ok, vr, vc);
+    if (slot < (KRS ? nrs : nw)) stage_row<T, HD>(Ks, kb, kst, tok, slot, half, geo.D);
+    if (slot < (KRS ? nw : nrs)) stage_row<T, HD>(Ks + 64 * HD, vb, vst, tok, slot, half, geo.D);
+    if (half == 0 && slot < nw) stage_key_cols(geo, key_cols(meta, st), h, g2l, gk, ok, vr, vc);
   }
   sm90::cp_async_commit();
 }
@@ -275,6 +298,64 @@
   sm90::cp_async_wait<kStages - 2>();
   sm90::fence_proxy_async();
   __syncthreads();
+}
+
+template <typename T, int HD, bool DROP, int NW>
+__device__ __forceinline__ void fwd_round(const Geo& geo, const T* Qs, const T* Ks, const T* Vs, const KeyCols& kcol,
+                                          const float* tab, int b, int h, int R, int C, int piece, int pi, int epi, int ngp,
+                                          const Visit* vl, float (&m)[2], float (&lsum)[2], float (&oacc)[HD / 2]) {
+  constexpr int HH = HD / 2;
+  using WHD = sm90::Wg<T, HD>;
+  float s[NW / 2];
+  sm90::wg_fence();
+#pragma unroll
+  for (int kk = 0; kk < HD / 16; ++kk)
+    sm90::Wg<T, NW>::ss(s, sm90::desc(Qs, HD, kk), sm90::desc(Ks, HD, kk), kk > 0);
+  sm90::wg_commit();
+  sm90::wg_wait0();
+  sm90::reg_fence(s);
+  float mx[2] = {-INFINITY, -INFINITY};
+  const int gl = geo.g - pi * 64;
+  switch (epi) {
+    case 0: fwd_scores<false, false, NW>(s, mx, geo, kcol, tab, query_rows(geo, R, C, piece), gl); break;
+    case 1: fwd_scores<false, true, NW>(s, mx, geo, kcol, tab, query_rows(geo, R, C, piece), gl); break;
+    case 2: fwd_scores<true, false, NW>(s, mx, geo, kcol, tab, query_rows(geo, R, C, piece), gl); break;
+    default: fwd_scores<true, true, NW>(s, mx, geo, kcol, tab, query_rows(geo, R, C, piece), gl); break;
+  }
+  float corr[2];
+#pragma unroll
+  for (int e = 0; e < 2; ++e) {
+    mx[e] = fmaxf(mx[e], __shfl_xor_sync(0xffffffffu, mx[e], 1));
+    mx[e] = fmaxf(mx[e], __shfl_xor_sync(0xffffffffu, mx[e], 2));
+    const float mn = fmaxf(m[e], mx[e]);
+    corr[e] = (mn == -INFINITY) ? 1.f : __expf(m[e] - mn);
+    m[e] = mn;
+    lsum[e] *= corr[e];
+  }
+#pragma unroll
+  for (int i = 0; i < NW / 2; ++i) {
+    const int e = (i >> 1) & 1;
+    const float p = (m[e] == -INFINITY) ? 0.f : __expf(s[i] - m[e]);
+    s[i] = p;
+    lsum[e] += p;
+  }
+#pragma unroll
+  for (int i = 0; i < HH; ++i) oacc[i] *= corr[(i >> 1) & 1];
+  if constexpr (DROP) {
+    uint32_t drow[2];
+    drop_rows(geo, R, C, piece, drow);
+    drop_key_piece<NW>(s, geo, drow, drop_col_base(geo, vl, ngp, pi), 2u * (uint32_t)(b * geo.H + h), 1.f);
+  }
+  constexpr int NK = (NW + 15) / 16;
+  uint32_t a[NK][4];
+#pragma unroll
+  for (int kk = 0; kk < NK; ++kk) to_a_frag<T, NW>(s, kk, a[kk]);
+  sm90::wg_fence();
+#pragma unroll
+  for (int kk = 0; kk < NK; ++kk) WHD::rs(oacc, a[kk], sm90::desc_mn(Vs, HD, kk), 1);
+  sm90::wg_commit();
+  sm90::wg_wait0();
+  sm90::reg_fence(oacc);
 }
 
 template <typename T, int HD, typename TO, bool DROP = false>
@@ -282,14 +363,14 @@
 wg_fwd_local(Geo geo, T4 q, T4 k, T4 v, T4 o, float* __restrict__ lse, const float* __restrict__ table,
              const float* __restrict__ g2l) {
   constexpr int HH = HD / 2, TILE = 64 * HD;
-  using W64 = sm90::Wg<T, 64>;
   using WHD = sm90::Wg<T, HD>;
   extern __shared__ __align__(128) unsigned char smem_raw[];
   T* Qs = reinterpret_cast<T*>(smem_raw);
   T* ring = Qs + TILE;
   unsigned char* meta = reinterpret_cast<unsigned char*>(ring + 2 * kStages * TILE);
   Visit* vl = reinterpret_cast<Visit*>(meta + kStages * kKeyCols);
-  float* tab = reinterpret_cast<float*>(vl + 9);
+  int* widths = reinterpret_cast<int*>(vl + 9);
+  float* tab = reinterpret_cast<float*>(widths + kStages);
   const int tabn = geo.has_bias ? (4 * geo.w - 1) * (4 * geo.w - 1) : 0;
 
   const Cta cid = decode(geo, blockIdx.x);
@@ -316,62 +397,18 @@
   __syncthreads();
 #pragma unroll
   for (int p = 0; p < kStages - 1; ++p)
-    issue_key_piece<T, HD>(geo, p, npieces, ngp, vl, wk, ring, meta, kb, k.st, vb, v.st, h, g2l);
+    issue_key_piece<T, HD, false, !DROP>(geo, p, npieces, ngp, vl, wk, widths, ring, meta, kb, k.st, vb, v.st, h, g2l);
   for (int pi = 0; pi < npieces; ++pi) {
     ring_wait();
-    issue_key_piece<T, HD>(geo, pi + kStages - 1, npieces, ngp, vl, wk, ring, meta, kb, k.st, vb, v.st, h, g2l);
+    issue_key_piece<T, HD, false, !DROP>(geo, pi + kStages - 1, npieces, ngp, vl, wk, widths, ring, meta, kb, k.st, vb, v.st, h, g2l);
     const int st = pi % kStages;
     const T* Ks = ring + st * 2 * TILE;
     const T* Vs = Ks + TILE;
     const KeyCols kcol = key_cols(meta, st);
-    float s[32];
-    sm90::wg_fence();
-#pragma unroll
-    for (int kk = 0; kk < HD / 16; ++kk) W64::ss(s, sm90::desc(Qs, HD, kk), sm90::desc(Ks, HD, kk), kk > 0);
-    sm90::wg_commit();
-    sm90::wg_wait0();
-    sm90::reg_fence(s);
-    float mx[2] = {-INFINITY, -INFINITY};
-    const int gl = geo.g - pi * 64;
-    switch (epi) {
-      case 0: fwd_scores<false, false>(s, mx, geo, kcol, tab, query_rows(geo, R, C, cid.piece), gl); break;
-      case 1: fwd_scores<false, true>(s, mx, geo, kcol, tab, query_rows(geo, R, C, cid.piece), gl); break;
-      case 2: fwd_scores<true, false>(s, mx, geo, kcol, tab, query_rows(geo, R, C, cid.piece), gl); break;
-      default: fwd_scores<true, true>(s, mx, geo, kcol, tab, query_rows(geo, R, C, cid.piece), gl); break;
-    }
-    float corr[2];
-#pragma unroll
-    for (int e = 0; e < 2; ++e) {
-      mx[e] = fmaxf(mx[e], __shfl_xor_sync(0xffffffffu, mx[e], 1));
-      mx[e] = fmaxf(mx[e], __shfl_xor_sync(0xffffffffu, mx[e], 2));
-      const float mn = fmaxf(m[e], mx[e]);
-      corr[e] = (mn == -INFINITY) ? 1.f : __expf(m[e] - mn);
-      m[e] = mn;
-      lsum[e] *= corr[e];
-    }
-#pragma unroll
-    for (int i = 0; i < 32; ++i) {
-      const int e = (i >> 1) & 1;
-      const float p = (m[e] == -INFINITY) ? 0.f : __expf(s[i] - m[e]);
-      s[i] = p;
-      lsum[e] += p;
-    }
-#pragma unroll
-    for (int i = 0; i < HH; ++i) oacc[i] *= corr[(i >> 1) & 1];
-    if constexpr (DROP) {
-      uint32_t drow[2];
-      drop_rows(geo, R, C, cid.piece, drow);
-      drop_key_piece(s, geo, drow, drop_col_base(geo, vl, ngp, pi), 2u * (uint32_t)(b * geo.H + h), 1.f);
-    }
-    uint32_t a[4][4];
-#pragma unroll
-    for (int kk = 0; kk < 4; ++kk) to_a_frag<T>(s, kk, a[kk]);
-    sm90::wg_fence();
-#pragma unroll
-    for (int kk = 0; kk < 4; ++kk) WHD::rs(oacc, a[kk], sm90::desc_mn(Vs, HD, kk), 1);
-    sm90::wg_commit();
-    sm90::wg_wait0();
-    sm90::reg_fence(oacc);
+#define ROUND(NW) fwd_round<T, HD, DROP, NW>(geo, Qs, Ks, Vs, kcol, tab, b, h, R, C, cid.piece, pi, epi, ngp, vl, m, lsum, oacc)
+    if constexpr (DROP) ROUND(64);
+    else VIL_BY_WIDTH(widths[st], ROUND)
+#undef ROUND
   }
   const QRows qrow = query_rows(geo, R, C, cid.piece);
 #pragma unroll
@@ -386,12 +423,52 @@
   }
 }
 
+template <typename T, int HD, bool DROP, int NW>
+__device__ __forceinline__ void dq_round(const Geo& geo, const T* Qs, const T* Gs, const T* Ks, const T* Vs, const KeyCols& kcol,
+                                         const float* tab, int b, int h, int R, int C, int piece, int pi, int epi, int ngp,
+                                         const Visit* vl, const QRows& qrow, const float (&lse_r)[2], const float (&del_r)[2],
+                                         float* __restrict__ d_table, float (&dqacc)[HD / 2]) {
+  using WHD = sm90::Wg<T, HD>;
+  using WNW = sm90::Wg<T, NW>;
+  float s[NW / 2], dp[NW / 2];
+  sm90::wg_fence();
+#pragma unroll
+  for (int kk = 0; kk < HD / 16; ++kk) WNW::ss(s, sm90::desc(Qs, HD, kk), sm90::desc(Ks, HD, kk), kk > 0);
+#pragma unroll
+  for (int kk = 0; kk < HD / 16; ++kk) WNW::ss(dp, sm90::desc(Gs, HD, kk), sm90::desc(Vs, HD, kk), kk > 0);
+  sm90::wg_commit();
+  sm90::wg_wait0();
+  sm90::reg_fence(s);
+  sm90::reg_fence(dp);
+  const int gl = geo.g - pi * 64;
+  if constexpr (DROP) {
+    uint32_t drow[2];
+    drop_rows(geo, R, C, piece, drow);
+    drop_key_piece<NW>(dp, geo, drow, drop_col_base(geo, vl, ngp, pi), 2u * (uint32_t)(b * geo.H + h), geo.drop_scale);
+  }
+  switch (epi) {
+    case 0: dq_scores<false, false, NW>(s, dp, geo, kcol, tab, qrow, gl, lse_r, del_r, d_table, h); break;
+    case 1: dq_scores<false, true, NW>(s, dp, geo, kcol, tab, qrow, gl, lse_r, del_r, d_table, h); break;
+    case 2: dq_scores<true, false, NW>(s, dp, geo, kcol, tab, qrow, gl, lse_r, del_r, d_table, h); break;
+    default: dq_scores<true, true, NW>(s, dp, geo, kcol, tab, qrow, gl, lse_r, del_r, d_table, h); break;
+  }
+  constexpr int NK = (NW + 15) / 16;
+  uint32_t a[NK][4];
+#pragma unroll
+  for (int kk = 0; kk < NK; ++kk) to_a_frag<T, NW>(s, kk, a[kk]);
+  sm90::wg_fence();
+#pragma unroll
+  for (int kk = 0; kk < NK; ++kk) WHD::rs(dqacc, a[kk], sm90::desc_mn(Ks, HD, kk), 1);
+  sm90::wg_commit();
+  sm90::wg_wait0();
+  sm90::reg_fence(dqacc);
+}
+
 template <typename T, int HD, typename TO, bool DROP = false>
-__global__ void __launch_bounds__(kThreads)
+__global__ void __launch_bounds__(kThreads, HD <= 32 && !DROP ? 4 : 3)
 wg_bwd_dq(Geo geo, T4 q, T4 k, T4 v, T4 d_o, T4 dq, const float* __restrict__ lse, const float* __restrict__ delta,
           const float* __restrict__ table, const float* __restrict__ g2l, float* __restrict__ d_table) {
   constexpr int HH = HD / 2, TILE = 64 * HD;
-  using W64 = sm90::Wg<T, 64>;
   using WHD = sm90::Wg<T, HD>;
   extern __shared__ __align__(128) unsigned char smem_raw[];
   T* Qs = reinterpret_cast<T*>(smem_raw);
@@ -399,7 +476,8 @@
   T* ring = Gs + TILE;
   unsigned char* meta = reinterpret_cast<unsigned char*>(ring + 2 * kStages * TILE);
   Visit* vl = reinterpret_cast<Visit*>(meta + kStages * kKeyCols);
-  float* tab = reinterpret_cast<float*>(vl + 9);
+  int* widths = reinterpret_cast<int*>(vl + 9);
+  float* tab = reinterpret_cast<float*>(widths + kStages);
   const int tabn = geo.has_bias ? (4 * geo.w - 1) * (4 * geo.w - 1) : 0;
 
   const Cta cid = decode(geo, blockIdx.x);
@@ -438,45 +516,17 @@
   __syncthreads();
 #pragma unroll
   for (int p = 0; p < kStages - 1; ++p)
-    issue_key_piece<T, HD>(geo, p, npieces, ngp, vl, wk, ring, meta, kb, k.st, vb, v.st, h, g2l);
+    issue_key_piece<T, HD, true>(geo, p, npieces, ngp, vl, wk, widths, ring, meta, kb, k.st, vb, v.st, h, g2l);
   for (int pi = 0; pi < npieces; ++pi) {
     ring_wait();
-    issue_key_piece<T, HD>(geo, pi + kStages - 1, npieces, ngp, vl, wk, ring, meta, kb, k.st, vb, v.st, h, g2l);
+    issue_key_piece<T, HD, true>(geo, pi + kStages - 1, npieces, ngp, vl, wk, widths, ring, meta, kb, k.st, vb, v.st, h, g2l);
     const int st = pi % kStages;
     const T* Ks = ring + st * 2 * TILE;
     const T* Vs = Ks + TILE;
     const KeyCols kcol = key_cols(meta, st);
-    float s[32], dp[32];
-    sm90::wg_fence();
-#pragma unroll
-    for (int kk = 0; kk < HD / 16; ++kk) W64::ss(s, sm90::desc(Qs, HD, kk), sm90::desc(Ks, HD, kk), kk > 0);
-#pragma unroll
-    for (int kk = 0; kk < HD / 16; ++kk) W64::ss(dp, sm90::desc(Gs, HD, kk), sm90::desc(Vs, HD, kk), kk > 0);
-    sm90::wg_commit();
-    sm90::wg_wait0();
-    sm90::reg_fence(s);
-    sm90::reg_fence(dp);
-    const int gl = geo.g - pi * 64;
-    if constexpr (DROP) {
-      uint32_t drow[2];
-      drop_rows(geo, R, C, cid.piece, drow);
-      drop_key_piece(dp, geo, drow, drop_col_base(geo, vl, ngp, pi), 2u * (uint32_t)(b * geo.H + h), geo.drop_scale);
-    }
-    switch (epi) {
-      case 0: dq_scores<false, false>(s, dp, geo, kcol, tab, qrow, gl, lse_r, del_r, d_table, h); break;
-      case 1: dq_scores<false, true>(s, dp, geo, kcol, tab, qrow, gl, lse_r, del_r, d_table, h); break;
-      case 2: dq_scores<true, false>(s, dp, geo, kcol, tab, qrow, gl, lse_r, del_r, d_table, h); break;
-      default: dq_scores<true, true>(s, dp, geo, kcol, tab, qrow, gl, lse_r, del_r, d_table, h); break;
-    }
-    uint32_t a[4][4];
-#pragma unroll
-    for (int kk = 0; kk < 4; ++kk) to_a_frag<T>(s, kk, a[kk]);
-    sm90::wg_fence();
-#pragma unroll
-    for (int kk = 0; kk < 4; ++kk) WHD::rs(dqacc, a[kk], sm90::desc_mn(Ks, HD, kk), 1);
-    sm90::wg_commit();
-    sm90::wg_wait0();
-    sm90::reg_fence(dqacc);
+#define ROUND(NW) dq_round<T, HD, DROP, NW>(geo, Qs, Gs, Ks, Vs, kcol, tab, b, h, R, C, cid.piece, pi, epi, ngp, vl, qrow, lse_r, del_r, d_table, dqacc)
+    VIL_BY_WIDTH(widths[st], ROUND)
+#undef ROUND
   }
 #pragma unroll
   for (int e = 0; e < 2; ++e) {
@@ -577,11 +627,11 @@
   return (geo.has_bias ? 3 : 0) + (geo.exact == 1 ? 1 : geo.exact == -1 ? 2 : 0);
 }
 
-template <bool RPE, int MASK>
-__device__ __forceinline__ void dkv_probs(float (&s)[32], float (&dp)[32], const Geo& geo, const QueryCols& qc, const float* tab,
-                                          const KRows& kr) {
-#pragma unroll
-  for (int i = 0; i < 32; ++i) {
+template <bool RPE, int MASK, int NW>
+__device__ __forceinline__ void dkv_probs(float (&s)[NW / 2], float (&dp)[NW / 2], const Geo& geo, const QueryCols& qc,
+                                          const float* tab, const KRows& kr) {
+#pragma unroll
+  for (int i = 0; i < NW / 2; ++i) {
     const int e = (i >> 1) & 1, j = acc_col(i);
     float x = fmaf(geo.scale, s[i], RPE ? tab[qc.tix[j] - kr.tb[e]] : 0.f) - qc.lse[j];
     if (MASK == 1 && (abs(qc.qr[j] - kr.kr[e]) > geo.w || abs(qc.qc[j] - kr.kc[e]) > geo.w)) x = -INFINITY;
@@ -592,45 +642,15 @@
   }
 }
 
-template <typename T, int HD, typename TO, bool DROP = false>
-__global__ void __launch_bounds__(kThreads, (HD <= 32 ? 4 : 3) - (DROP ? 1 : 0))
-wg_bwd_dkv(Geo geo, T4 q, T4 k, T4 v, T4 d_o, T4 dk, T4 dv, const float* __restrict__ lse, const float* __restrict__ delta,
-           const float* __restrict__ table) {
-  constexpr int HH = HD / 2, TILE = 64 * HD;
-  using W64 = sm90::Wg<T, 64>;
+template <typename T, int HD, bool DROP, int NW>
+__device__ __forceinline__ void dkv_walk(const Geo& geo, const T4& q, const T4& d_o, const float* __restrict__ lse,
+                                         const float* __restrict__ delta, const T* Ks, const T* Vs, T* ring,
+                                         unsigned char* meta, int cols, const Visit* vl, const int* kpos, const float* tab,
+                                         int b, int h, int KR, int KC, int piece, long long bh, int npieces, int epi, int slot,
+                                         float (&dkacc)[HD / 2], float (&dvacc)[HD / 2]) {
+  constexpr int TILE = 64 * HD;
+  using WNW = sm90::Wg<T, NW>;
   using WHD = sm90::Wg<T, HD>;
-  extern __shared__ __align__(128) unsigned char smem_raw[];
-  T* Ks = reinterpret_cast<T*>(smem_raw);
-  T* Vs = Ks + TILE;
-  T* ring = Vs + TILE;
-  unsigned char* meta = reinterpret_cast<unsigned char*>(ring + 2 * kStages * TILE);
-  const int cols = (int)query_cols_bytes(DROP);
-  Visit* vl = reinterpret_cast<Visit*>(meta + kStages * cols);
-  int* kpos = reinterpret_cast<int*>(vl + 9);
-  float* tab = reinterpret_cast<float*>(kpos + 64);
-  const int tw = 4 * geo.w - 1;
-  const int tabn = geo.has_bias ? tw * tw : 0;
-
-  const Cta cid = decode(geo, blockIdx.x);
-  const int b = cid.b, h = cid.h, KR = cid.R, KC = cid.C;
-  const int tid = threadIdx.x, slot = tid >> 1, half = tid & 1;
-  const int w = geo.w, D = geo.D;
-  const long long bh = (long long)b * geo.H + h;
-  for (int i = tid; i < tabn; i += kThreads) tab[i] = table[(long long)i * geo.H + h];
-  {
-    const int lk = cid.piece * 64 + slot;
-    const int ar = KR * w + lk / w, ac = KC * w + lk % w;
-    const long long tokk = (lk < geo.w2 && ar < geo.nx && ac < geo.ny) ? geo.g + (long long)ar * geo.ny + ac : -1;
-    stage_row<T, HD>(Ks, row_ptr<T>(k, b, h, 0), k.st, tokk, slot, half, D);
-    stage_row<T, HD>(Vs, row_ptr<T>(v, b, h, 0), v.st, tokk, slot, half, D);
-    if (half == 0) kpos[slot] = key_pos(geo, cid.piece, slot);
-  }
-  float dkacc[HH], dvacc[HH];
-#pragma unroll
-  for (int i = 0; i < HH; ++i) { dkacc[i] = 0.f; dvacc[i] = 0.f; }
-
-  const int npieces = visit_list(geo, KR, KC, -1, vl) * geo.npc;
-  const int epi = query_epilogue(geo);
   SlotWalk wk(geo, slot);
   __syncthreads();
 #pragma unroll
@@ -648,50 +668,95 @@
     uint32_t keep = 0;
     if constexpr (DROP) {
       const int vi = qp / geo.npc;
-      const uint32_t c0 = (uint32_t)(geo.g + vl[vi].oi * geo.w2 + cid.piece * 64), sid = 2u * (uint32_t)(b * geo.H + h);
+      const uint32_t c0 = (uint32_t)(geo.g + vl[vi].oi * geo.w2 + piece * 64), sid = 2u * (uint32_t)(b * geo.H + h);
 #pragma unroll 1
-      for (int i = 0; i < 32; ++i)
+      for (int i = 0; i < NW / 2; ++i)
         keep |= (uint32_t)drop_keep(geo, (uint32_t)qcol.tok[acc_col(i)], c0 + (uint32_t)acc_row(i), sid) << i;
     }
-    float s[32], dp[32];
+    float s[NW / 2], dp[NW / 2];
     sm90::wg_fence();
 #pragma unroll
-    for (int kk = 0; kk < HD / 16; ++kk) W64::ss(s, sm90::desc(Ks, HD, kk), sm90::desc(Qs, HD, kk), kk > 0);
-#pragma unroll
-    for (int kk = 0; kk < HD / 16; ++kk) W64::ss(dp, sm90::desc(Vs, HD, kk), sm90::desc(Gs, HD, kk), kk > 0);
+    for (int kk = 0; kk < HD / 16; ++kk) WNW::ss(s, sm90::desc(Ks, HD, kk), sm90::desc(Qs, HD, kk), kk > 0);
+#pragma unroll
+    for (int kk = 0; kk < HD / 16; ++kk) WNW::ss(dp, sm90::desc(Vs, HD, kk), sm90::desc(Gs, HD, kk), kk > 0);
     sm90::wg_commit();
     sm90::wg_wait0();
     sm90::reg_fence(s);
     sm90::reg_fence(dp);
     if constexpr (DROP) {
 #pragma unroll
-      for (int i = 0; i < 32; ++i) dp[i] = (keep >> i) & 1u ? dp[i] * geo.drop_scale : 0.f;
+      for (int i = 0; i < NW / 2; ++i) dp[i] = (keep >> i) & 1u ? dp[i] * geo.drop_scale : 0.f;
     }
     switch (epi) {
-      case 0: dkv_probs<false, 0>(s, dp, geo, qcol, tab, key_rows(geo, KR, KC, kpos)); break;
-      case 1: dkv_probs<false, 1>(s, dp, geo, qcol, tab, key_rows(geo, KR, KC, kpos)); break;
-      case 2: dkv_probs<false, 2>(s, dp, geo, qcol, tab, key_rows(geo, KR, KC, kpos)); break;
-      case 3: dkv_probs<true, 0>(s, dp, geo, qcol, tab, key_rows(geo, KR, KC, kpos)); break;
-      case 4: dkv_probs<true, 1>(s, dp, geo, qcol, tab, key_rows(geo, KR, KC, kpos)); break;
-      default: dkv_probs<true, 2>(s, dp, geo, qcol, tab, key_rows(geo, KR, KC, kpos)); break;
+      case 0: dkv_probs<false, 0, NW>(s, dp, geo, qcol, tab, key_rows(geo, KR, KC, kpos)); break;
+      case 1: dkv_probs<false, 1, NW>(s, dp, geo, qcol, tab, key_rows(geo, KR, KC, kpos)); break;
+      case 2: dkv_probs<false, 2, NW>(s, dp, geo, qcol, tab, key_rows(geo, KR, KC, kpos)); break;
+      case 3: dkv_probs<true, 0, NW>(s, dp, geo, qcol, tab, key_rows(geo, KR, KC, kpos)); break;
+      case 4: dkv_probs<true, 1, NW>(s, dp, geo, qcol, tab, key_rows(geo, KR, KC, kpos)); break;
+      default: dkv_probs<true, 2, NW>(s, dp, geo, qcol, tab, key_rows(geo, KR, KC, kpos)); break;
     }
     if constexpr (DROP) {
 #pragma unroll
-      for (int i = 0; i < 32; ++i) s[i] = (keep >> i) & 1u ? s[i] * geo.drop_scale : 0.f;
+      for (int i = 0; i < NW / 2; ++i) s[i] = (keep >> i) & 1u ? s[i] * geo.drop_scale : 0.f;
     }
-    uint32_t ap[4][4], ad[4][4];
-#pragma unroll
-    for (int kk = 0; kk < 4; ++kk) { to_a_frag<T>(s, kk, ap[kk]); to_a_frag<T>(dp, kk, ad[kk]); }
+    constexpr int NK = (NW + 15) / 16;
+    uint32_t ap[NK][4], ad[NK][4];
+#pragma unroll
+    for (int kk = 0; kk < NK; ++kk) { to_a_frag<T, NW>(s, kk, ap[kk]); to_a_frag<T, NW>(dp, kk, ad[kk]); }
     sm90::wg_fence();
 #pragma unroll
-    for (int kk = 0; kk < 4; ++kk) WHD::rs(dvacc, ap[kk], sm90::desc_mn(Gs, HD, kk), 1);
-#pragma unroll
-    for (int kk = 0; kk < 4; ++kk) WHD::rs(dkacc, ad[kk], sm90::desc_mn(Qs, HD, kk), 1);
+    for (int kk = 0; kk < NK; ++kk) WHD::rs(dvacc, ap[kk], sm90::desc_mn(Gs, HD, kk), 1);
+#pragma unroll
+    for (int kk = 0; kk < NK; ++kk) WHD::rs(dkacc, ad[kk], sm90::desc_mn(Qs, HD, kk), 1);
     sm90::wg_commit();
     sm90::wg_wait0();
     sm90::reg_fence(dvacc);
     sm90::reg_fence(dkacc);
   }
+}
+
+template <typename T, int HD, typename TO, bool DROP = false>
+__global__ void __launch_bounds__(kThreads, (HD <= 32 ? 4 : 3) - (DROP ? 1 : 0))
+wg_bwd_dkv(Geo geo, T4 q, T4 k, T4 v, T4 d_o, T4 dk, T4 dv, const float* __restrict__ lse, const float* __restrict__ delta,
+           const float* __restrict__ table) {
+  constexpr int HH = HD / 2, TILE = 64 * HD;
+  extern __shared__ __align__(128) unsigned char smem_raw[];
+  T* Ks = reinterpret_cast<T*>(smem_raw);
+  T* Vs = Ks + TILE;
+  T* ring = Vs + TILE;
+  unsigned char* meta = reinterpret_cast<unsigned char*>(ring + 2 * kStages * TILE);
+  const int cols = (int)query_cols_bytes(DROP);
+  Visit* vl = reinterpret_cast<Visit*>(meta + kStages * cols);
+  int* kpos = reinterpret_cast<int*>(vl + 9);
+  float* tab = reinterpret_cast<float*>(kpos + 64);
+  const int tw = 4 * geo.w - 1;
+  const int tabn = geo.has_bias ? tw * tw : 0;
+
+  const Cta cid = decode(geo, blockIdx.x);
+  const int b = cid.b, h = cid.h, KR = cid.R, KC = cid.C;
+  const int tid = threadIdx.x, slot = tid >> 1, half = tid & 1;
+  const int w = geo.w, D = geo.D;
+  const long long bh = (long long)b * geo.H + h;
+  for (int i = tid; i < tabn; i += kThreads) tab[i] = table[(long long)i * geo.H + h];
+  {
+    const int lk = cid.piece * 64 + slot;
+    const int ar = KR * w + lk / w, ac = KC * w + lk % w;
+    const long long tokk = (lk < geo.w2 && ar < geo.nx && ac < geo.ny) ? geo.g + (long long)ar * geo.ny + ac : -1;
+    stage_row<T, HD>(Ks, row_ptr<T>(k, b, h, 0), k.st, tokk, slot, half, D);
+    stage_row<T, HD>(Vs, row_ptr<T>(v, b, h, 0), v.st, tokk, slot, half, D);
+    if (half == 0) kpos[slot] = key_pos(geo, cid.piece, slot);
+  }
+  float dkacc[HH], dvacc[HH];
+#pragma unroll
+  for (int i = 0; i < HH; ++i) { dkacc[i] = 0.f; dvacc[i] = 0.f; }
+
+  const int npieces = visit_list(geo, KR, KC, -1, vl) * geo.npc;
+  const int epi = query_epilogue(geo);
+#define WALK(NW) dkv_walk<T, HD, DROP, NW>(geo, q, d_o, lse, delta, Ks, Vs, ring, meta, cols, vl, kpos, tab, b, h, KR, KC, \
+                                           cid.piece, bh, npieces, epi, slot, dkacc, dvacc)
+  if (geo.npc == 1 && geo.w2 <= 56 && !geo.full_pieces) WALK(56);
+  else WALK(64);
+#undef WALK
   const KRows krow = key_rows(geo, KR, KC, kpos);
 #pragma unroll
   for (int e = 0; e < 2; ++e) {
```

Result: no change. 3832 (median of 6 runs) (+0.7%).
